# monniert/differentiable-blocksworld

Measured on AMD Instinct MI355X. Metric: rendered views/sec (fwd+bwd) per node, DTU 400x300 K=10 blocks, higher is better.
Workload: dtype f32; 1 GPU; DTU-scan24-like synthetic: 49 views/GPU/step, 400x300, 10 superquadric blocks + ground + sky dome, faces_per_pixel=10, 256^2 textures, coarse phase (sigma=1e-4, opacity noise, decimated textures), MSE+parsimony+TV+overlap, Adam; LPIPS excluded; views_per_gpu=49, n_blocks=10, faces_per_pixel=10, txt_size=256, parallelism=one GPU: all views on it, no collective, nranks=1

## Files before the change

### differentiable-blocksworld_amd/csrc/project_clip.hip

```cpp
#include "dbw_common.h"
#include "camera_math.h"
#include "shade_common.h"
#include "raster_bin.h"
#include "step_kernels.h"
#include "texture_body.h"
#include "../../include/dbw_hip.h"

using namespace dbw;

namespace {

constexpr int NT = 256;

__device__ __forceinline__ void store_tri(float *dst, f3 a, f3 b, f3 c) {
    dst[0] = a.x; dst[1] = a.y; dst[2] = a.z;
    dst[3] = b.x; dst[4] = b.y; dst[5] = b.z;
    dst[6] = c.x; dst[7] = c.y; dst[8] = c.z;
}

__global__ __launch_bounds__(NT) void project_clip_fwd_kernel(
    const float *__restrict__ verts, const int *__restrict__ faces, const float *__restrict__ R,
    const float *__restrict__ T, const float *__restrict__ Kmat, int V, int F, float eps, int zc_on, float zc,
    int persp, float *__restrict__ fvc, int *__restrict__ first_idx, int *__restrict__ num_faces,
    int *__restrict__ c2o, int *__restrict__ neighbor, int *__restrict__ code, float *__restrict__ cw) {
    __shared__ int s_wcnt[NT / DBW_WAVE];
    const int b = blockIdx.x, tid = threadIdx.x, lane = tid & 63, wv = tid >> 6;
    Cam cam;
    load_cam(R, T, Kmat, b, cam);
    const long long base_out = (long long)b * 2 * F;
    int running = 0;
    for (int f0 = 0; f0 < F; f0 += NT) {
        const int f = f0 + tid;
        ClippedFace cf;
        cf.emit = 0;
        if (f < F) {
            f3 p[3];
#pragma unroll
            for (int i = 0; i < 3; ++i) p[i] = project(verts + (long long)faces[f * 3 + i] * 3, cam, eps).ndc;
            clip_face(p, zc_on, zc, persp, cf);
        }
        const int emit = cf.emit;
        const unsigned long long m1 = __ballot(emit >= 1), m2 = __ballot(emit == 2);
        const unsigned long long lower = (1ull << lane) - 1ull;
        const int prefix = __popcll(m1 & lower) + __popcll(m2 & lower);
        if (lane == 0) s_wcnt[wv] = __popcll(m1) + __popcll(m2);
        __syncthreads();
        int woff = 0, tot = 0;
#pragma unroll
        for (int w = 0; w < NT / DBW_WAVE; ++w) { const int c = s_wcnt[w]; if (w < wv) woff += c; tot += c; }
        const int slot = running + woff + prefix;
        if (emit >= 1) {
            const long long o = base_out + slot;
            store_tri(fvc + o * 9, cf.t0[0], cf.t0[1], cf.t0[2]);
            c2o[o] = f; neighbor[o] = emit == 2 ? (int)(o + 1) : -1; code[o] = cf.code0; cw[o * 2] = cf.w2; cw[o * 2 + 1] = cf.w3;
            if (emit == 2) {
                store_tri(fvc + (o + 1) * 9, cf.t1[0], cf.t1[1], cf.t1[2]);
                c2o[o + 1] = f; neighbor[o + 1] = (int)o; code[o + 1] = cf.code1; cw[(o + 1) * 2] = cf.w2; cw[(o + 1) * 2 + 1] = cf.w3;
            }
        }
        running += tot;
        __syncthreads();
    }
    if (tid == 0) { first_idx[b] = (int)base_out; num_faces[b] = running; }
}

constexpr int BWD_SLOTS = 8;
template <bool LDS_TABLE>
__device__ __forceinline__ void project_clip_bwd_body(
    const float *__restrict__ verts, const int *__restrict__ faces, const float *__restrict__ R,
    const float *__restrict__ T, const float *__restrict__ Kmat, int B, int V, int F, float eps, float zc, int persp,
    const int *__restrict__ num_faces, const int *__restrict__ c2o, const int *__restrict__ code,
    const float *__restrict__ cw, const float *__restrict__ gfvc, float *gverts, float *s_acc, int blk) {
    const int lane = threadIdx.x & 63;
    if (LDS_TABLE) {
        for (int i = threadIdx.x; i < V * 3; i += NT) s_acc[i] = 0.f;
        __syncthreads();
    }
    constexpr int WAVES = NT / DBW_WAVE, ITERS = LDS_TABLE ? BWD_SLOTS / WAVES : 1;
    for (int it = 0; it < ITERS; ++it) {
    const int j = LDS_TABLE ? blk * BWD_SLOTS + it * WAVES + (threadIdx.x >> 6) : blk * WAVES + (threadIdx.x >> 6);
    if (j >= 2 * F) break;
    for (int b0 = 0; b0 < B; b0 += DBW_WAVE) {
        const int b = b0 + lane;
        bool act = b < B && j < num_faces[b];
        const long long o = (long long)(act ? b : 0) * 2 * F + j;
        float g[9];
        if (act) {
            bool any = false;
#pragma unroll
            for (int i = 0; i < 9; ++i) { g[i] = gfvc[o * 9 + i]; any |= (g[i] != 0.f); }
            act = any;
        }
        int f = -1, vi[3] = {0, 0, 0};
        float gw[9] = {0.f, 0.f, 0.f, 0.f, 0.f, 0.f, 0.f, 0.f, 0.f};
        if (act) {
            Cam cam;
            load_cam(R, T, Kmat, b, cam);
            f = c2o[o];
            const int cd = code[o];
            vi[0] = faces[f * 3]; vi[1] = faces[f * 3 + 1]; vi[2] = faces[f * 3 + 2];
            f3 gv[3] = {{0.f, 0.f, 0.f}, {0.f, 0.f, 0.f}, {0.f, 0.f, 0.f}};
            const f3 ga{g[0], g[1], g[2]}, gb{g[3], g[4], g[5]}, gc{g[6], g[7], g[8]};
            if (cd < 0) {
                gv[0] = ga; gv[1] = gb; gv[2] = gc;
            } else {
                const int i1 = cd & 3, kind = cd >> 2;
                const f3 q0 = project(verts + (long long)vi[0] * 3, cam, eps).ndc, q1 = project(verts + (long long)vi[1] * 3, cam, eps).ndc,
                         q2 = project(verts + (long long)vi[2] * 3, cam, eps).ndc;
                const f3 P1 = i1 == 0 ? q0 : (i1 == 1 ? q1 : q2), P2 = i1 == 0 ? q1 : (i1 == 1 ? q2 : q0),
                         P3 = i1 == 0 ? q2 : (i1 == 1 ? q0 : q1);
                const float w2 = cw[o * 2], w3 = cw[o * 2 + 1];
                f3 g1{0.f, 0.f, 0.f}, g2{0.f, 0.f, 0.f}, g3{0.f, 0.f, 0.f};
                if (kind == 0) {
                    clip_point_bwd(P1, P2, zc, persp, w2, ga, g1, g2);
                    clip_point_bwd(P1, P3, zc, persp, w3, gb, g1, g3);
                    g1.x += gc.x; g1.y += gc.y; g1.z += gc.z;
                } else if (kind == 1) {
                    clip_point_bwd(P1, P2, zc, persp, w2, ga, g1, g2);
                    g2.x += gb.x; g2.y += gb.y; g2.z += gb.z;
                    clip_point_bwd(P1, P3, zc, persp, w3, gc, g1, g3);
                } else {
                    clip_point_bwd(P1, P3, zc, persp, w3, ga, g1, g3);
                    g2.x += gb.x; g2.y += gb.y; g2.z += gb.z;
                    g3.x += gc.x; g3.y += gc.y; g3.z += gc.z;
                }
                gv[0] = i1 == 0 ? g1 : (i1 == 1 ? g3 : g2);
                gv[1] = i1 == 0 ? g2 : (i1 == 1 ? g1 : g3);
                gv[2] = i1 == 0 ? g3 : (i1 == 1 ? g2 : g1);
            }
#pragma unroll
            for (int i = 0; i < 3; ++i)
                if (gv[i].x != 0.f || gv[i].y != 0.f || gv[i].z != 0.f) {
                    const f3 w = vertex_bwd(verts, vi[i], cam, eps, gv[i]);
                    gw[i * 3] = w.x; gw[i * 3 + 1] = w.y; gw[i * 3 + 2] = w.z;
                }
        }
        const unsigned long long am = __ballot(act);
        if (am == 0ull) continue;
        const int leader = __ffsll((long long)am) - 1;
        const int f0 = __shfl(f, leader, 64);
        if (__popcll(am) >= 4 && __ballot(act && f == f0) == am) {
            float s[9];
#pragma unroll
            for (int c = 0; c < 9; ++c) s[c] = wave_sum_dpp(gw[c]);
            if (lane == leader) {
#pragma unroll
                for (int c = 0; c < 9; ++c)
                    if (s[c] != 0.f) {
                        if (LDS_TABLE) atomicAdd(&s_acc[vi[c / 3] * 3 + (c % 3)], s[c]);
                        else unsafeAtomicAdd(gverts + (long long)vi[c / 3] * 3 + (c % 3), s[c]);
                    }
            }
        } else if (act) {
#pragma unroll
            for (int c = 0; c < 9; ++c)
                if (gw[c] != 0.f) {
                    if (LDS_TABLE) atomicAdd(&s_acc[vi[c / 3] * 3 + (c % 3)], gw[c]);
                    else unsafeAtomicAdd(gverts + (long long)vi[c / 3] * 3 + (c % 3), gw[c]);
                }
        }
    }
    }
    if (LDS_TABLE) {
        __syncthreads();
        for (int i = threadIdx.x; i < V * 3; i += NT) {
            const float v = s_acc[i];
            if (v != 0.f) unsafeAtomicAdd(gverts + i, v);
        }
    }
}

template <bool LDS_TABLE>
__global__ __launch_bounds__(NT) void project_clip_bwd_kernel(
    const float *__restrict__ verts, const int *__restrict__ faces, const float *__restrict__ R,
    const float *__restrict__ T, const float *__restrict__ Kmat, int B, int V, int F, float eps, float zc, int persp,
    const int *__restrict__ num_faces, const int *__restrict__ c2o, const int *__restrict__ code,
    const float *__restrict__ cw, const float *__restrict__ gfvc, float *__restrict__ gverts) {
    extern __shared__ float s_acc[];
    project_clip_bwd_body<LDS_TABLE>(verts, faces, R, T, Kmat, B, V, F, eps, zc, persp, num_faces, c2o, code, cw, gfvc, gverts, s_acc, blockIdx.x);
}

template <bool LDS_TABLE>
__global__ __launch_bounds__(NT) void clip_bwd_tex_kernel(const ClipBwdArgs C, const dbw_texture_set t, int nclip) {
    extern __shared__ float s_acc[];
    if ((int)blockIdx.x < nclip)
        project_clip_bwd_body<LDS_TABLE>(C.verts, C.faces, C.R, C.T, C.Kmat, C.B, C.V, C.F, C.eps, C.zc, C.persp, C.num_faces, C.c2o, C.code, C.cw, C.gfvc,
                                         C.gverts, s_acc, blockIdx.x);
    else
        texture_prep_bwd_body(t.texture, t.n, t.h, t.w, t.decim, t.grad_maps, t.grad_sig, t.grad_texture, (long long)blockIdx.x - nclip,
                              (long long)gridDim.x - nclip);
}

template <bool CACHED>
__global__ __launch_bounds__(NT) void scene_setup_kernel(const SceneSetupArgs A) {
    __shared__ int s_wcnt[NT / DBW_WAVE];
    extern __shared__ float s_ndc[];
    if (A.sync_flag && blockIdx.x == 0 && blockIdx.y == 0 && blockIdx.z == 0 && threadIdx.x == 0)
        __hip_atomic_store(A.sync_flag, A.sync_val, __ATOMIC_RELEASE, __HIP_MEMORY_SCOPE_AGENT);
    const SceneGeom &G = A.sc[A.scene0 + blockIdx.z];
    const int chunk = blockIdx.x, b = blockIdx.y, tid = threadIdx.x, lane = tid & 63, wv = tid >> 6;
    const int F = G.F, nchunks = (F + NT - 1) / NT;
    if (chunk >= nchunks) return;
    if (G.hdr && chunk == 0 && b == 0)
        for (int i = tid; i < G.nhdr; i += NT) G.hdr[i] = 0;
    Cam cam;
    load_cam(A.R, A.T, A.Kmat, b, cam);
    const long long base_out = (long long)b * 2 * F;
    const int f = chunk * NT + tid;
    int vi[3] = {0, 0, 0};
    if (f < F) { vi[0] = G.faces[f * 3]; vi[1] = G.faces[f * 3 + 1]; vi[2] = G.faces[f * 3 + 2]; }
    if (CACHED) {
        for (int v = tid; v < G.V; v += NT) {
            const f3 q = project(G.verts + (long long)v * 3, cam, G.cam_eps).ndc;
            s_ndc[v * 3] = q.x; s_ndc[v * 3 + 1] = q.y; s_ndc[v * 3 + 2] = q.z;
        }
        __syncthreads();
    }
    int before = 0;
    for (int g = tid; g < chunk * NT; g += NT) {
        const int i0 = G.faces[g * 3], i1 = G.faces[g * 3 + 1], i2 = G.faces[g * 3 + 2];
        float z0, z1, z2;
        if (CACHED) { z0 = s_ndc[i0 * 3 + 2]; z1 = s_ndc[i1 * 3 + 2]; z2 = s_ndc[i2 * 3 + 2]; }
        else { z0 = view_z(G.verts + (long long)i0 * 3, cam); z1 = view_z(G.verts + (long long)i1 * 3, cam); z2 = view_z(G.verts + (long long)i2 * 3, cam); }
        before += clip_emit_count(z0, z1, z2, G.zc_on, G.zc);
    }
#pragma unroll
    for (int o = 32; o > 0; o >>= 1) before += __shfl_xor(before, o, 64);
    if (lane == 0) s_wcnt[wv] = before;
    __syncthreads();
    int running = 0;
#pragma unroll
    for (int w = 0; w < NT / DBW_WAVE; ++w) running += s_wcnt[w];
    __syncthreads();
    ClippedFace cf;
    cf.emit = 0;
    if (f < F) {
        f3 p[3];
#pragma unroll
        for (int i = 0; i < 3; ++i) {
            if (CACHED) p[i] = f3{s_ndc[vi[i] * 3], s_ndc[vi[i] * 3 + 1], s_ndc[vi[i] * 3 + 2]};
            else p[i] = project(G.verts + (long long)vi[i] * 3, cam, G.cam_eps).ndc;
        }
        clip_face(p, G.zc_on, G.zc, G.persp, cf);
    }
    const int emit = cf.emit;
    const unsigned long long m1 = __ballot(emit >= 1), m2 = __ballot(emit == 2);
    const unsigned long long lower = (1ull << lane) - 1ull;
    const int prefix = __popcll(m1 & lower) + __popcll(m2 & lower);
    if (lane == 0) s_wcnt[wv] = __popcll(m1) + __popcll(m2);
    __syncthreads();
    int woff = 0, tot = 0;
#pragma unroll
    for (int w = 0; w < NT / DBW_WAVE; ++w) { const int c = s_wcnt[w]; if (w < wv) woff += c; tot += c; }
    const int slot = running + woff + prefix;
    FaceRec *recs = (FaceRec *)G.recs;
    ShadeRec *srec = (ShadeRec *)G.srec;
#pragma unroll
    for (int t = 0; t < 2; ++t) {
        if (t >= emit) break;
        const long long o = base_out + slot + t;
        const f3 a = t == 0 ? cf.t0[0] : cf.t1[0], bq = t == 0 ? cf.t0[1] : cf.t1[1], cq = t == 0 ? cf.t0[2] : cf.t1[2];
        const float p9[9] = {a.x, a.y, a.z, bq.x, bq.y, bq.z, cq.x, cq.y, cq.z};
        const int nbr = emit == 2 ? (int)(t == 0 ? o + 1 : o - 1) : -1, cd = t == 0 ? cf.code0 : cf.code1;
#pragma unroll
        for (int i = 0; i < 9; ++i) G.fvc[o * 9 + i] = p9[i];
        G.c2o[o] = f; G.neighbor[o] = nbr; G.code[o] = cd; G.cw[o * 2] = cf.w2; G.cw[o * 2 + 1] = cf.w3;
        FaceRec r;
        float box[4];
        make_face_rec(p9, G.margin, 0, nbr, r, box);
        G.bbox[o] = make_float4(box[0], box[1], box[2], box[3]);
        recs[o] = r;
        if (srec) {
            ShadeRec sr;
            const float *uv = G.face_uvs + (long long)f * 6;
#pragma unroll
            for (int i = 0; i < 6; ++i) sr.uv[i] = uv[i];
            sr.j = f; sr.cd = cd; sr.w2 = cf.w2; sr.w3 = cf.w3;
            sr.map = G.face_map[f];
            sr.fa = G.map_alpha ? G.map_alpha[sr.map] : 1.f;
            const int *md = G.map_desc + sr.map * 8;
            sr.off = md[0]; sr.hw = (md[1] << 16) | md[2]; sr.pads = (md[3] << 16) | md[4]; sr.sh = md[5];
            srec[o] = sr;
        }
    }
    if (chunk == nchunks - 1 && tid == 0) {
        G.first_idx[b] = (int)base_out;
        G.num_faces[b] = running + tot;
        if (srec && b == 0 && running + tot == 0) {
            ShadeRec sr;
#pragma unroll
            for (int i = 0; i < 6; ++i) sr.uv[i] = 0.f;
            sr.j = 0; sr.cd = -1; sr.w2 = sr.w3 = 0.f; sr.map = 0; sr.fa = 0.f; sr.off = 0; sr.hw = (1 << 16) | 1; sr.pads = 0; sr.sh = 0;
            srec[0] = sr;
        }
    }
}

}

int dbw::launch_clip_bwd_tex(const ClipBwdArgs &C, const dbw_texture_set &t, hipStream_t s) {
    DBW_REQUIRE(C.verts && C.faces && C.R && C.T && C.Kmat && C.num_faces && C.c2o && C.code && C.cw && C.gfvc && C.gverts, "null pointer");
    DBW_REQUIRE(C.B > 0 && C.V > 0 && C.F > 0, "bad size");
    DBW_REQUIRE(t.texture && t.grad_maps && t.grad_texture && t.n > 0 && t.h > 0 && t.w > 0 && t.decim >= 1, "bad texture set");
    const long long work = (long long)t.n * t.h * t.w * 3;
    long long ntex = (work + NT - 1) / NT;
    if (ntex > 4096) ntex = 4096;
    const bool table = (size_t)C.V * 3 * sizeof(float) <= 48 * 1024;
    const int nclip = table ? (2 * C.F + BWD_SLOTS - 1) / BWD_SLOTS : (2 * C.F + NT / DBW_WAVE - 1) / (NT / DBW_WAVE);
    if (table)
        hipLaunchKernelGGL(clip_bwd_tex_kernel<true>, dim3((unsigned)(nclip + ntex)), dim3(NT), (size_t)C.V * 3 * sizeof(float), s, C, t, nclip);
    else
        hipLaunchKernelGGL(clip_bwd_tex_kernel<false>, dim3((unsigned)(nclip + ntex)), dim3(NT), 0, s, C, t, nclip);
    return dbw_check_launch("clip_bwd_tex_kernel");
}

int dbw::launch_scene_setup(const SceneSetupArgs &A, hipStream_t s) {
    DBW_REQUIRE(A.R && A.T && A.Kmat && A.B > 0, "bad argument");
    int chunks = 0;
    DBW_REQUIRE(A.scene0 >= 0 && A.nscenes >= 1 && A.scene0 + A.nscenes <= 2, "bad scene range");
    for (int i = A.scene0; i < A.scene0 + A.nscenes; ++i) {
        const SceneGeom &G = A.sc[i];
        DBW_REQUIRE(G.verts && G.faces && G.fvc && G.first_idx && G.num_faces && G.c2o && G.neighbor && G.code && G.cw && G.bbox && G.recs, "null pointer");
        DBW_REQUIRE(G.V > 0 && G.F > 0 && (long long)A.B * 2 * G.F < 0x7fffffffLL && (!G.zc_on || G.zc > 0.f), "bad size / z_clip");
        DBW_REQUIRE(!G.srec || (G.face_uvs && G.face_map && G.map_desc), "null pointer");
        chunks = max(chunks, (G.F + NT - 1) / NT);
    }
    int vmax = 0;
    for (int i = A.scene0; i < A.scene0 + A.nscenes; ++i) vmax = max(vmax, A.sc[i].V);
    if ((size_t)vmax * 12 <= 40 * 1024)
        hipLaunchKernelGGL(scene_setup_kernel<true>, dim3((unsigned)chunks, (unsigned)A.B, (unsigned)A.nscenes), dim3(NT), (size_t)vmax * 12, s, A);
    else
        hipLaunchKernelGGL(scene_setup_kernel<false>, dim3((unsigned)chunks, (unsigned)A.B, (unsigned)A.nscenes), dim3(NT), 0, s, A);
    return dbw_check_launch("scene_setup_kernel");
}

extern "C" int dbw_project_clip_fwd(const float *verts_world, const int32_t *faces, const float *R, const float *T,
                                    const float *Kmat, int B, int V, int F, float eps, int z_clip_enabled,
                                    float z_clip, int perspective_correct, float *face_verts_c, int32_t *first_idx,
                                    int32_t *num_faces, int32_t *c2o, int32_t *neighbor, int32_t *clip_code,
                                    float *clip_w, dbw_stream_t stream) {
    DBW_REQUIRE(verts_world && faces && R && T && Kmat && face_verts_c && first_idx && num_faces && c2o && neighbor &&
                    clip_code && clip_w, "null pointer");
    DBW_REQUIRE(B >= 0 && V > 0 && F > 0, "bad size");
    DBW_REQUIRE((long long)B * 2 * F < 0x7fffffffLL, "B*2F overflows int32 face indices");
    DBW_REQUIRE(!z_clip_enabled || z_clip > 0.f, "z_clip must be > 0");
    if (B == 0) return DBW_OK;
    hipLaunchKernelGGL(project_clip_fwd_kernel, dim3(B), dim3(NT), 0, (hipStream_t)stream, verts_world, faces, R, T,
                       Kmat, V, F, eps, z_clip_enabled, z_clip, perspective_correct, face_verts_c, first_idx,
                       num_faces, c2o, neighbor, clip_code, clip_w);
    return dbw_check_launch("project_clip_fwd_kernel");
}

extern "C" int dbw_project_clip_bwd(const float *verts_world, const int32_t *faces, const float *R, const float *T,
                                    const float *Kmat, int B, int V, int F, float eps, float z_clip,
                                    int perspective_correct, const int32_t *num_faces, const int32_t *c2o,
                                    const int32_t *clip_code, const float *clip_w, const float *grad_face_verts_c,
                                    float *grad_verts_world, dbw_stream_t stream) {
    DBW_REQUIRE(verts_world && faces && R && T && Kmat && num_faces && c2o && clip_code && clip_w &&
                    grad_face_verts_c && grad_verts_world, "null pointer");
    DBW_REQUIRE(B >= 0 && V > 0 && F > 0, "bad size");
    if (B == 0) return DBW_OK;
    if ((size_t)V * 3 * sizeof(float) <= 48 * 1024)
        hipLaunchKernelGGL(project_clip_bwd_kernel<true>, dim3((2 * F + BWD_SLOTS - 1) / BWD_SLOTS), dim3(NT), (size_t)V * 3 * sizeof(float),
                           (hipStream_t)stream, verts_world, faces, R, T, Kmat, B, V, F, eps, z_clip, perspective_correct, num_faces, c2o,
                           clip_code, clip_w, grad_face_verts_c, grad_verts_world);
    else
        hipLaunchKernelGGL(project_clip_bwd_kernel<false>, dim3((2 * F + NT / DBW_WAVE - 1) / (NT / DBW_WAVE)), dim3(NT), 0, (hipStream_t)stream,
                           verts_world, faces, R, T, Kmat, B, V, F, eps, z_clip, perspective_correct, num_faces, c2o,
                           clip_code, clip_w, grad_face_verts_c, grad_verts_world);
    return dbw_check_launch("project_clip_bwd_kernel");
}
```

### differentiable-blocksworld_amd/csrc/step_kernels.h

```cpp
#pragma once
#include <hip/hip_runtime.h>
#include <stdint.h>

#include "../../include/dbw_hip.h"

namespace dbw {
struct RasterWorkspace;

constexpr int STEP_MAX_SETS = 4;
struct StepTextureSets { dbw_texture_set s[STEP_MAX_SETS]; };

struct PrologueArgs {
    StepTextureSets tex; int nsets;
    const float *alpha_logit, *noise;
    float noise_scale, thresh;
    int nb;
    float *alpha, *alpha_full;
    int *keep;
    unsigned long long seed, rng_step;
    const float *sq_eps, *S, *R6, *T, *trig;
    int nv;
    float ratio, scale_min, S_world;
    const float *Rw, *Tw;
    float *blk_verts;
    float *sq_local;
    const float *ground_base; int ngv;
    const float *R6g, *Tg;
    float *ground_verts;
    float *zero0; int nzero0;
};
int launch_step_prologue(const PrologueArgs &P, hipStream_t s);

struct SceneGeom {
    const float *verts; const int *faces; int V, F;
    float cam_eps; int zc_on; float zc; int persp;
    float *fvc; int *first_idx, *num_faces, *c2o, *neighbor, *code; float *cw;
    float margin;
    float4 *bbox; void *recs;
    int *hdr; int nhdr;
    void *srec; const float *face_uvs; const int *face_map, *map_desc; const float *map_alpha;
};
struct SceneSetupArgs { SceneGeom sc[2]; const float *R, *T, *Kmat; int B; int scene0, nscenes;
                        unsigned *sync_flag; unsigned sync_val; };
int launch_scene_setup(const SceneSetupArgs &A, hipStream_t s);

struct SceneBinsArgs {
    struct One {
        const float4 *bbox; const void *recs; const int *first_idx, *num_faces;
        int *list, *count; unsigned *mask;
        int cells; int2 *cell; int *pool; int pool_cap; int *hdr; int *rank;
        int *dom;
    } sc[2];
    int B, H, W, nx, ny;
    int scene0, nscenes;
    StepTextureSets tex; int tex_sets, tex_z;
};
int launch_scene_bins(const SceneBinsArgs &A, hipStream_t s);
int dbw_launch_work_scatter(const RasterWorkspace &L, int N, int H, int W, hipStream_t s, unsigned *sync_flag = nullptr, unsigned sync_val = 0);

struct RegulariserArgs {
    const float *u; int npts;
    unsigned long long seed, rng_step;
    const float *sq_eps, *S, *R6, *T, *alpha_full;
    int nb;
    float ratio, scale_min, inv_temp, thresh, overlap_scale;
    float pars_eps, pars_scale;
    float *loss_parsimony, *loss_overlap;
    float *g_sq_eps, *g_S, *g_R6, *g_T, *g_alpha_full;
    float *ws;
    unsigned *ticket;
};
int launch_regularisers(const RegulariserArgs &A, hipStream_t s);

struct BlocksTailArgs {
    const float *sq_eps, *S, *R6, *T, *sq_local; const int *keep; int nb, nv; float scale_min, S_world; const float *Rw;
    const float *g_verts;
    float *g_sq_eps, *g_S, *g_R6, *g_T;
    const float *alpha, *g_alpha_parts, *g_alpha_full; int alpha_parts; float *g_logit;
    const float *void_raised; float *void_flag;
};
int launch_blocks_tail(const BlocksTailArgs &A, hipStream_t s);

struct ClipBwdArgs {
    const float *verts; const int *faces; const float *R, *T, *Kmat; int B, V, F; float eps, zc; int persp;
    const int *num_faces, *c2o, *code; const float *cw, *gfvc; float *gverts;
};
int launch_clip_bwd_tex(const ClipBwdArgs &C, const dbw_texture_set &tex, hipStream_t s);

struct AdamTailArgs {
    float *param, *grad, *exp_avg, *exp_avg_sq; const int64_t *group_end; const float *lr; int ngroups;
    float beta1, beta2, eps; int step;
    void *zero_buf; int64_t zero_bytes, hole_begin, hole_end;
    dbw_texture_set tex[2]; int ntex;
    const float *void_raised; float *void_flag;
};
bool adam_tail_fits(const AdamTailArgs &A);
int launch_adam_tail(const AdamTailArgs &A, hipStream_t s);

struct EnvFoldHost {
    const RasterWorkspace *ws; const int *first_idx, *num_faces; const float *maps; float bg[3];
    int *p2f; float *uvj;
};
int render_fwd_fused_mse_fold(const float *face_verts_c, const int32_t *first_idx, const int32_t *num_faces, const int32_t *neighbor,
                              const int32_t *c2o, const int32_t *clip_code, const float *clip_w, int Fc_stride, const float *face_uvs,
                              const int32_t *face_map, const int32_t *map_desc, const float *maps, const float *faces_alpha, int alpha_len, int N,
                              int64_t F_total, int H, int W, int K, int F, float sigma, float blur_radius, int perspective_correct,
                              const float *background3, int32_t *pix_to_face, float *bary, float *dists, void *workspace, size_t workspace_bytes,
                              const float *target, float mse_scale, float *loss_partial, float *grad_fg, float *grad_env, const EnvFoldHost &fold,
                              float *rec_out, const float *grad_rec, hipStream_t stream);

int render_bwd_fused_signal(const int32_t *pix_to_face, const float *bary, const float *dists, const int32_t *c2o, const int32_t *clip_code,
                            const float *clip_w, int Fc_stride, const float *face_uvs, const int32_t *face_map, const int32_t *map_desc, const float *maps,
                            const float *faces_alpha, int alpha_len, int N, int H, int W, int K, int F, float sigma, const float *background3,
                            const float *grad_image, const float *face_verts_c, int perspective_correct, int detach_bary, float *grad_maps,
                            float *grad_faces_alpha, float *grad_face_verts_c, int lds_aggregate, int frag_layout, const int32_t *bin_base,
                            int32_t *bin_cursor, void *bin_records, int bin_cap, const uint32_t *bin_layout, int const_geometry_faces,
                            const float *grad_scale, int image_layout, dbw_stream_t stream, unsigned *sync_flag, unsigned sync_val);

}
```

### differentiable-blocksworld_amd/csrc/texture.hip

```cpp
#include "dbw_common.h"
#include "loss_math.h"
#include "texture_body.h"
#include "step_kernels.h"
#include "../../include/dbw_hip.h"

#include <string.h>
#include <algorithm>

using namespace dbw;

namespace {

constexpr int NT = 256;

__device__ __forceinline__ float sigmoidf(float x) { return 1.f / (1.f + expf(-x)); }

__device__ __forceinline__ float block_sum(float v, float *s_red) {
    v = wave_sum(v);
    const int lane = threadIdx.x & 63, wv = threadIdx.x >> 6;
    __syncthreads();
    if (lane == 0) s_red[wv] = v;
    __syncthreads();
    float t = 0.f;
#pragma unroll
    for (int w = 0; w < NT / DBW_WAVE; ++w) t += s_red[w];
    return t;
}

__global__ __launch_bounds__(256) void texture_prep_fwd_kernel(const float *__restrict__ tex, int n, int h, int w, int d,
                                                               float *__restrict__ maps, float *__restrict__ sig) {
    texture_prep_fwd_body(tex, n, h, w, d, maps, sig, blockIdx.x, gridDim.x);
}

constexpr int MAX_SETS = 4;
struct TextureSets { dbw_texture_set s[MAX_SETS]; };

__global__ __launch_bounds__(256) void texture_prep_fwd_sets_kernel(const TextureSets S) {
    const dbw_texture_set &t = S.s[blockIdx.y];
    texture_prep_fwd_body(t.texture, t.n, t.h, t.w, t.decim, t.maps, t.sig, blockIdx.x, gridDim.x);
}

__global__ void texture_prep_bwd_kernel(const float *__restrict__ tex, int n, int h, int w, int d,
                                        const float *__restrict__ gmaps, const float *__restrict__ gsig,
                                        float *__restrict__ gtex) {
    texture_prep_bwd_body(tex, n, h, w, d, gmaps, gsig, gtex, blockIdx.x, gridDim.x);
}

__global__ void texture_prep_bwd_sets_kernel(const TextureSets S) {
    const dbw_texture_set &t = S.s[blockIdx.y];
    texture_prep_bwd_body(t.texture, t.n, t.h, t.w, t.decim, t.grad_maps, t.grad_sig, t.grad_texture, blockIdx.x, gridDim.x);
}

__device__ __forceinline__ void tv_l2sq_body(const float *__restrict__ m, int n, int h, int w, int wrap,
                                             float scale, float *__restrict__ loss, float *__restrict__ gm, float *s_red) {
    const float sx = 1.f / ((float)h * (float)(w - 1 + (wrap ? 1 : 0)));
    const float sy = 1.f / ((float)(h - 1) * (float)w);
    float part = 0.f;
    for (int row = blockIdx.y; row < n * h; row += gridDim.y) {
        const int y = row % h;
        const float *r = m + (long long)row * w * 3;
        for (int x = blockIdx.x * NT + threadIdx.x; x < w; x += gridDim.x * NT) {
            float g3[3];
            part += tv_l2sq_texel(r, x, y, w, h, wrap, sx, sy, g3);
            if (gm) {
#pragma unroll
                for (int c = 0; c < 3; ++c) gm[((long long)row * w + x) * 3 + c] = scale * g3[c];
            }
        }
    }
    const float tot = block_sum(part, s_red);
    if (threadIdx.x == 0 && tot != 0.f) unsafeAtomicAdd(loss, scale * tot);
}

__global__ __launch_bounds__(NT) void tv_l2sq_kernel(const float *__restrict__ m, int n, int h, int w, int wrap,
                                                     float scale, float *__restrict__ loss, float *__restrict__ gm) {
    __shared__ float s_red[NT / DBW_WAVE];
    tv_l2sq_body(m, n, h, w, wrap, scale, loss, gm, s_red);
}

__global__ __launch_bounds__(NT) void tv_l2sq_sets_kernel(const TextureSets S, float *__restrict__ loss) {
    __shared__ float s_red[NT / DBW_WAVE];
    const dbw_texture_set &t = S.s[blockIdx.z];
    tv_l2sq_body(t.sig, t.n, t.h, t.w, t.wrap_x, t.tv_scale, loss, t.grad_sig_out, s_red);
}

constexpr int CNT = 1024;
__global__ __launch_bounds__(CNT) void composite_mse_kernel(const float *__restrict__ fg, const float *__restrict__ env,
                                                           const float *__restrict__ img, int N, long long plane,
                                                           float scale, const float *__restrict__ scale_dev, float *__restrict__ rec,
                                                           float *__restrict__ loss, float *__restrict__ gfg,
                                                           float *__restrict__ genv) {
    __shared__ float s_red[CNT / DBW_WAVE];
    const long long total = (long long)N * plane;
    float part = 0.f;
    const float loss_scale = scale;
    if (scale_dev) scale *= scale_dev[0];
    for (long long i0 = (long long)blockIdx.x * CNT; i0 < total; i0 += (long long)gridDim.x * CNT) {
        const long long i = i0 + threadIdx.x;
        if (i < total) {
            const long long n = i / plane, p = i % plane;
            const float *f = fg + n * 4 * plane + p, *e = env + n * 4 * plane + p;
            const float *t = img ? img + n * 3 * plane + p : nullptr;
            const float mask = f[3 * plane];
            const float fc3[3] = {f[0], f[plane], f[2 * plane]}, ec3[3] = {e[0], e[plane], e[2 * plane]};
            const float t3[3] = {t ? t[0] : 0.f, t ? t[plane] : 0.f, t ? t[2 * plane] : 0.f};
            float rec3[3], gf3[3], ge3[3], gmask = 0.f;
            part += composite_mse_pixel(fc3, mask, ec3, t3, t != nullptr, 2.f * scale, rec3, gf3, ge3, gmask);
#pragma unroll
            for (int c = 0; c < 3; ++c) {
                if (rec) rec[n * 3 * plane + c * plane + p] = rec3[c];
                if (gfg) { gfg[n * 4 * plane + c * plane + p] = gf3[c]; genv[n * 4 * plane + c * plane + p] = ge3[c]; }
            }
            if (gfg) { gfg[n * 4 * plane + 3 * plane + p] = gmask; genv[n * 4 * plane + 3 * plane + p] = 0.f; }
        }
    }
    part = wave_sum(part);
    if ((threadIdx.x & 63) == 0) s_red[threadIdx.x >> 6] = part;
    __syncthreads();
    if (threadIdx.x == 0 && loss) {
        float tot = 0.f;
        for (int w = 0; w < CNT / DBW_WAVE; ++w) tot += s_red[w];
        unsafeAtomicAdd(loss, tot * loss_scale);
    }
}

__global__ void adam_kernel(float *__restrict__ p, const float *__restrict__ g, float *__restrict__ m,
                            float *__restrict__ v, long long n, float step_size, float beta1, float beta2, float eps,
                            float bc2_sqrt) {
    for (long long i = (long long)blockIdx.x * blockDim.x + threadIdx.x; i < n; i += (long long)gridDim.x * blockDim.x) {
        adam_update(p[i], g[i], m[i], v[i], step_size, beta1, beta2, eps, bc2_sqrt);
    }
}

struct AdamGroups { long long end[MAX_SETS]; float step_size[MAX_SETS]; };

__global__ void adam_groups_kernel(float *__restrict__ p, const float *__restrict__ g, float *__restrict__ m, float *__restrict__ v,
                                   long long n, const AdamGroups G, float beta1, float beta2, float eps, float bc2_sqrt,
                                   uint4 *__restrict__ zero_buf, long long zero_vec, const float *__restrict__ skip_flag) {
    if (skip_flag && *skip_flag != 0.f) n = 0;
    for (long long i = (long long)blockIdx.x * blockDim.x + threadIdx.x; i < n; i += (long long)gridDim.x * blockDim.x) {
        float step_size = G.step_size[0];
#pragma unroll
        for (int k = 1; k < MAX_SETS; ++k) step_size = i >= G.end[k - 1] ? G.step_size[k] : step_size;
        adam_update(p[i], g[i], m[i], v[i], step_size, beta1, beta2, eps, bc2_sqrt);
    }
    for (long long i = (long long)blockIdx.x * blockDim.x + threadIdx.x; i < zero_vec; i += (long long)gridDim.x * blockDim.x)
        zero_buf[i] = make_uint4(0u, 0u, 0u, 0u);
}

__device__ __forceinline__ float group_step_size(const AdamGroups &G, long long i) {
    float step_size = G.step_size[0];
#pragma unroll
    for (int k = 1; k < MAX_SETS; ++k) step_size = i >= G.end[k - 1] ? G.step_size[k] : step_size;
    return step_size;
}

struct AdamTex { const float *tex; const float *gsig; float *gmaps; int n, h, w, d; long long off; };
struct AdamTailK {
    float *p, *g, *m, *v; long long n; AdamGroups G; float beta1, beta2, eps, bc2_sqrt;
    uint4 *zero_buf; long long zero_vec, hole_lo, hole_hi;
    AdamTex t[2]; int ntex, clear_maps, nenv;
    long long skip_lo[2], skip_len[2];
    const float *void_raised; float *void_flag;
};

__device__ __forceinline__ void adam_tex_set(const AdamTailK &A, const AdamTex &t, bool skip, long long etid, long long neth) {
    if (t.d <= 1) {
        const long long total = (long long)t.n * t.h * t.w * 3;
        for (long long i = etid; i < total; i += neth) {
            const float s = tex_sigmoid(t.tex[i]);
            float g = t.gmaps[i];
            if (A.clear_maps) t.gmaps[i] = 0.f;
            if (t.gsig) g += t.gsig[i];
            const float gt = g * s * (1.f - s);
            const long long o = t.off + i;
            A.g[o] = gt;
            if (!skip) adam_update(A.p[o], gt, A.m[o], A.v[o], group_step_size(A.G, o), A.beta1, A.beta2, A.eps, A.bc2_sqrt);
        }
        return;
    }
    const float inv = 1.f / (float)(t.d * t.d);
    const int ch_ = t.h / t.d, cw_ = t.w / t.d, lane = threadIdx.x & 63;
    const long long cells = (long long)t.n * ch_ * cw_;
    for (long long c = etid >> 6; c < cells; c += neth >> 6) {
        const int m = (int)(c / ((long long)ch_ * cw_));
        const int r = (int)(c % ((long long)ch_ * cw_));
        const int cy = r / cw_, cx = r % cw_;
        const float gc[3] = {t.gmaps[c * 3], t.gmaps[c * 3 + 1], t.gmaps[c * 3 + 2]};
        for (int q = lane; q < t.d * t.d; q += 64) {
            const long long e = (((long long)m * t.h + cy * t.d + q / t.d) * t.w + cx * t.d + q % t.d) * 3;
#pragma unroll
            for (int ch = 0; ch < 3; ++ch) {
                const long long i = e + ch;
                const float s = tex_sigmoid(t.tex[i]);
                float g = gc[ch] * inv;
                if (t.gsig) g += t.gsig[i];
                const float gt = g * s * (1.f - s);
                const long long o = t.off + i;
                A.g[o] = gt;
                if (!skip) adam_update(A.p[o], gt, A.m[o], A.v[o], group_step_size(A.G, o), A.beta1, A.beta2, A.eps, A.bc2_sqrt);
            }
        }
        if (A.clear_maps && lane < 3) t.gmaps[c * 3 + lane] = 0.f;
    }
}

__global__ __launch_bounds__(NT) void adam_groups_tex_kernel(const AdamTailK A) {
    const bool skip = *A.void_raised != 0.f;
    if (blockIdx.x == 0 && threadIdx.x == 0 && A.void_flag) *A.void_flag = *A.void_raised;
    const long long tid = (long long)blockIdx.x * blockDim.x + threadIdx.x, nth = (long long)gridDim.x * blockDim.x;
    const long long neth = (long long)A.nenv * blockDim.x;
    if (tid < neth) {
        for (int k = 0; k < A.ntex; ++k) adam_tex_set(A, A.t[k], skip, tid, neth);
    } else if (!skip) {
        const long long rest = A.n - A.skip_len[0] - A.skip_len[1];
        for (long long j = tid - neth; j < rest; j += nth - neth) {
            long long i = j;
            if (i >= A.skip_lo[0]) i += A.skip_len[0];
            if (i >= A.skip_lo[1]) i += A.skip_len[1];
            adam_update(A.p[i], A.g[i], A.m[i], A.v[i], group_step_size(A.G, i), A.beta1, A.beta2, A.eps, A.bc2_sqrt);
        }
    }
    for (long long i = tid; i < A.zero_vec; i += nth)
        if (i < A.hole_lo || i >= A.hole_hi) A.zero_buf[i] = make_uint4(0u, 0u, 0u, 0u);
}

inline unsigned grid_for(long long work) {
    long long b = (work + NT - 1) / NT;
    if (b < 1) b = 1;
    if (b > 2048) b = 2048;
    return (unsigned)b;
}

}

extern "C" int dbw_texture_prep_fwd(const float *texture, int n, int h, int w, int decim, float *maps_out,
                                    float *sig_out, dbw_stream_t stream) {
    DBW_REQUIRE(texture && maps_out, "null pointer");
    DBW_REQUIRE(n > 0 && h > 0 && w > 0 && decim >= 1, "bad size");
    DBW_REQUIRE(decim == 1 || sig_out, "sig_out is required when decimating");
    DBW_REQUIRE(decim == 1 || (h % decim == 0 && w % decim == 0), "map size must be a multiple of the decimation factor");
    const long long work = decim > 1 ? (long long)n * (h / decim) * (w / decim) * 64 : (long long)n * h * w * 3;
    hipLaunchKernelGGL(texture_prep_fwd_kernel, dim3(grid_for(work)), dim3(NT), 0, (hipStream_t)stream, texture, n, h,
                       w, decim, maps_out, sig_out);
    return dbw_check_launch("texture_prep_fwd_kernel");
}

extern "C" int dbw_texture_prep_bwd(const float *texture, int n, int h, int w, int decim, const float *grad_maps,
                                    const float *grad_sig, float *grad_texture, dbw_stream_t stream) {
    DBW_REQUIRE(texture && grad_maps && grad_texture, "null pointer");
    DBW_REQUIRE(n > 0 && h > 0 && w > 0 && decim >= 1, "bad size");
    DBW_REQUIRE(decim == 1 || (h % decim == 0 && w % decim == 0), "map size must be a multiple of the decimation factor");
    const long long work = (long long)n * h * w * 3;
    hipLaunchKernelGGL(texture_prep_bwd_kernel, dim3(grid_for(work)), dim3(NT), 0, (hipStream_t)stream, texture, n, h,
                       w, decim, grad_maps, grad_sig, grad_texture);
    return dbw_check_launch("texture_prep_bwd_kernel");
}

extern "C" int dbw_tv_l2sq(const float *maps, int n, int h, int w, int wrap_x, float scale, float *loss,
                           float *grad_maps, dbw_stream_t stream) {
    DBW_REQUIRE(maps && loss, "null pointer");
    DBW_REQUIRE(n > 0 && h > 1 && w > 1, "bad size");
    const long long rows = (long long)n * h;
    hipLaunchKernelGGL(tv_l2sq_kernel, dim3((unsigned)((w + NT - 1) / NT), (unsigned)(rows < 512 ? rows : 512)), dim3(NT), 0,
                       (hipStream_t)stream, maps, n, h, w, wrap_x, scale, loss, grad_maps);
    return dbw_check_launch("tv_l2sq_kernel");
}

namespace {
int check_sets(const dbw_texture_set *sets, int nsets) {
    DBW_REQUIRE(sets && nsets >= 1 && nsets <= MAX_SETS, "1..4 texture sets");
    for (int i = 0; i < nsets; ++i) {
        const dbw_texture_set &t = sets[i];
        DBW_REQUIRE(t.n > 0 && t.h > 1 && t.w > 1 && t.decim >= 1, "bad size");
        DBW_REQUIRE(t.decim == 1 || (t.h % t.decim == 0 && t.w % t.decim == 0), "map size must be a multiple of the decimation factor");
    }
    return DBW_OK;
}
TextureSets pack_sets(const dbw_texture_set *sets, int nsets) {
    TextureSets S;
    for (int i = 0; i < MAX_SETS; ++i) S.s[i] = sets[i < nsets ? i : 0];
    return S;
}
AdamGroups adam_groups(const int64_t *group_end, const float *lr, int ngroups, float beta1, float beta2, int step, float &bc2_sqrt) {
    const long long n = group_end[ngroups - 1];
    const double bc1 = 1.0 - pow((double)beta1, step), bc2 = 1.0 - pow((double)beta2, step);
    AdamGroups G;
    for (int k = 0; k < MAX_SETS; ++k) {
        G.end[k] = k < ngroups ? group_end[k] : n;
        G.step_size[k] = (float)(lr[k < ngroups ? k : ngroups - 1] / bc1);
    }
    bc2_sqrt = (float)sqrt(bc2);
    return G;
}
}

extern "C" int dbw_texture_prep_fwd_sets(const dbw_texture_set *sets, int nsets, dbw_stream_t stream) {
    if (int rc = check_sets(sets, nsets)) return rc;
    long long work = 0;
    for (int i = 0; i < nsets; ++i) {
        const dbw_texture_set &t = sets[i];
        DBW_REQUIRE(t.texture && t.maps, "null pointer");
        DBW_REQUIRE(t.decim == 1 || t.sig, "sig is required when decimating");
        const long long wk = t.decim > 1 ? (long long)t.n * (t.h / t.decim) * (t.w / t.decim) * 64 : (long long)t.n * t.h * t.w * 3;
        work = wk > work ? wk : work;
    }
    hipLaunchKernelGGL(texture_prep_fwd_sets_kernel, dim3(grid_for(work), (unsigned)nsets), dim3(NT), 0, (hipStream_t)stream,
                       pack_sets(sets, nsets));
    return dbw_check_launch("texture_prep_fwd_sets_kernel");
}

extern "C" int dbw_texture_prep_bwd_sets(const dbw_texture_set *sets, int nsets, dbw_stream_t stream) {
    if (int rc = check_sets(sets, nsets)) return rc;
    long long work = 0;
    for (int i = 0; i < nsets; ++i) {
        const dbw_texture_set &t = sets[i];
        DBW_REQUIRE(t.texture && t.grad_maps && t.grad_texture, "null pointer");
        const long long wk = (long long)t.n * t.h * t.w * 3;
        work = wk > work ? wk : work;
    }
    hipLaunchKernelGGL(texture_prep_bwd_sets_kernel, dim3(grid_for(work), (unsigned)nsets), dim3(NT), 0, (hipStream_t)stream,
                       pack_sets(sets, nsets));
    return dbw_check_launch("texture_prep_bwd_sets_kernel");
}

extern "C" int dbw_tv_l2sq_sets(const dbw_texture_set *sets, int nsets, float *loss, dbw_stream_t stream) {
    if (int rc = check_sets(sets, nsets)) return rc;
    DBW_REQUIRE(loss, "null pointer");
    long long rows = 0;
    int w = 0;
    for (int i = 0; i < nsets; ++i) {
        DBW_REQUIRE(sets[i].sig, "null pointer");
        const long long r = (long long)sets[i].n * sets[i].h;
        rows = r > rows ? r : rows;
        w = sets[i].w > w ? sets[i].w : w;
    }
    hipLaunchKernelGGL(tv_l2sq_sets_kernel, dim3((unsigned)((w + NT - 1) / NT), (unsigned)(rows < 512 ? rows : 512), (unsigned)nsets),
                       dim3(NT), 0, (hipStream_t)stream, pack_sets(sets, nsets), loss);
    return dbw_check_launch("tv_l2sq_sets_kernel");
}

extern "C" int dbw_adam_step_groups(float *param, const float *grad, float *exp_avg, float *exp_avg_sq, const int64_t *group_end,
                                    const float *lr, int ngroups, float beta1, float beta2, float eps, int step, void *zero_buf,
                                    int64_t zero_bytes, const float *skip_flag, dbw_stream_t stream) {
    DBW_REQUIRE(param && grad && exp_avg && exp_avg_sq && group_end && lr, "null pointer");
    DBW_REQUIRE(zero_bytes >= 0 && (zero_bytes == 0 || (zero_buf && zero_bytes % 16 == 0 && ((uintptr_t)zero_buf & 15) == 0)),
                "zero_buf: 16-byte aligned, a multiple of 16 bytes");
    DBW_REQUIRE(ngroups >= 1 && ngroups <= MAX_SETS && step >= 1, "1..4 groups, step >= 1");
    for (int k = 0; k < ngroups; ++k) DBW_REQUIRE(group_end[k] >= (k ? group_end[k - 1] : 0), "group ends must not decrease");
    const long long n = group_end[ngroups - 1];
    if (n == 0) return DBW_OK;
    float bc2_sqrt;
    const AdamGroups G = adam_groups(group_end, lr, ngroups, beta1, beta2, step, bc2_sqrt);
    hipLaunchKernelGGL(adam_groups_kernel, dim3(grid_for(n)), dim3(NT), 0, (hipStream_t)stream, param, grad, exp_avg, exp_avg_sq, n, G,
                       beta1, beta2, eps, bc2_sqrt, (uint4 *)zero_buf, (long long)(zero_bytes / 16), skip_flag);
    return dbw_check_launch("adam_groups_kernel");
}

bool dbw::adam_tail_fits(const AdamTailArgs &A) {
    if (!A.param || !A.grad || !A.exp_avg || !A.exp_avg_sq || !A.group_end || !A.lr || !A.void_raised || A.ngroups < 1 || A.ngroups > MAX_SETS) return false;
    if (A.ntex < 0 || A.ntex > 2 || A.zero_bytes < 0 || A.zero_bytes % 16 || ((uintptr_t)A.zero_buf & 15)) return false;
    if (A.hole_begin < 0 || A.hole_begin > A.hole_end || A.hole_end > A.zero_bytes || A.hole_begin % 16 || A.hole_end % 16) return false;
    const long long n = A.group_end[A.ngroups - 1];
    const char *hb = (const char *)A.zero_buf + A.hole_begin, *he = (const char *)A.zero_buf + A.hole_end;
    long long lo[2] = {0, 0}, hi[2] = {0, 0};
    for (int k = 0; k < A.ntex; ++k) {
        const dbw_texture_set &t = A.tex[k];
        if (!t.texture || !t.grad_maps || !t.grad_texture || t.n < 1 || t.h < 1 || t.w < 1 || t.decim < 1 || t.h % t.decim || t.w % t.decim) return false;
        lo[k] = (long long)(t.grad_texture - A.grad);
        hi[k] = lo[k] + (long long)t.n * t.h * t.w * 3;
        if (t.grad_texture < A.grad || hi[k] > n || t.texture != A.param + lo[k]) return false;
        const char *mb = (const char *)t.grad_maps, *me = mb + (size_t)t.n * (t.h / t.decim) * (t.w / t.decim) * 3 * sizeof(float);
        const char *zb = (const char *)A.zero_buf, *ze = zb + A.zero_bytes;
        if (A.hole_end > A.hole_begin ? (mb < hb || me > he) : (mb < ze && me > zb)) return false;
    }
    return A.ntex < 2 || hi[0] <= lo[1] || hi[1] <= lo[0];
}

int dbw::launch_adam_tail(const AdamTailArgs &A, hipStream_t s) {
    DBW_REQUIRE(adam_tail_fits(A), "the texture sets must lie in the flat buffers, their maps' gradients in the hole of the arena");
    DBW_REQUIRE(A.step >= 1, "step >= 1");
    for (int k = 0; k < A.ngroups; ++k) DBW_REQUIRE(A.group_end[k] >= (k ? A.group_end[k - 1] : 0), "group ends must not decrease");
    AdamTailK K;
    memset(&K, 0, sizeof(K));
    K.p = A.param; K.g = A.grad; K.m = A.exp_avg; K.v = A.exp_avg_sq; K.n = A.group_end[A.ngroups - 1];
    K.G = adam_groups(A.group_end, A.lr, A.ngroups, A.beta1, A.beta2, A.step, K.bc2_sqrt);
    K.beta1 = A.beta1; K.beta2 = A.beta2; K.eps = A.eps;
    K.zero_buf = (uint4 *)A.zero_buf; K.zero_vec = A.zero_bytes / 16; K.hole_lo = A.hole_begin / 16; K.hole_hi = A.hole_end / 16;
    K.ntex = A.ntex; K.clear_maps = A.hole_end > A.hole_begin ? 1 : 0;
    for (int k = 0; k < A.ntex; ++k) {
        const dbw_texture_set &t = A.tex[k];
        K.t[k].tex = t.texture; K.t[k].gsig = t.grad_sig; K.t[k].gmaps = (float *)t.grad_maps;
        K.t[k].n = t.n; K.t[k].h = t.h; K.t[k].w = t.w; K.t[k].d = t.decim; K.t[k].off = (long long)(t.grad_texture - A.grad);
    }
    K.void_raised = A.void_raised; K.void_flag = A.void_flag;
    long long env = 0;
    for (int k = 0; k < 2; ++k) {
        K.skip_lo[k] = K.n; K.skip_len[k] = 0;
        if (k < A.ntex) { K.skip_lo[k] = K.t[k].off; K.skip_len[k] = (long long)K.t[k].n * K.t[k].h * K.t[k].w * 3; env += K.skip_len[k]; }
    }
    if (K.skip_lo[1] < K.skip_lo[0]) {
        std::swap(K.skip_lo[0], K.skip_lo[1]);
        std::swap(K.skip_len[0], K.skip_len[1]);
    }
    unsigned grid = grid_for(K.n);
    K.nenv = 0;
    if (A.ntex) {
        if (grid < 2) grid = 2;
        const double we = 10.0 / 7.0 * (double)env;
        const long long share = (long long)((double)grid * we / ((double)(K.n - env) + we) + 0.5);
        K.nenv = (int)std::min<long long>(grid - 1, std::max<long long>(1, share));
    }
    hipLaunchKernelGGL(adam_groups_tex_kernel, dim3(grid), dim3(NT), 0, s, K);
    return dbw_check_launch("adam_groups_tex_kernel");
}

extern "C" int dbw_debug_adam_tail(float *param, float *grad, float *exp_avg, float *exp_avg_sq, const int64_t *group_end, const float *lr,
                                   int ngroups, float beta1, float beta2, float eps, int step, void *zero_buf, int64_t zero_bytes,
                                   int64_t hole_begin, int64_t hole_end, const dbw_texture_set *sets, int nsets, const float *void_raised,
                                   float *void_flag, dbw_stream_t stream) {
    DBW_REQUIRE(nsets >= 0 && nsets <= 2 && (sets || nsets == 0), "0..2 texture sets");
    AdamTailArgs A;
    memset(&A, 0, sizeof(A));
    A.param = param; A.grad = grad; A.exp_avg = exp_avg; A.exp_avg_sq = exp_avg_sq; A.group_end = group_end; A.lr = lr; A.ngroups = ngroups;
    A.beta1 = beta1; A.beta2 = beta2; A.eps = eps; A.step = step;
    A.zero_buf = zero_buf; A.zero_bytes = zero_bytes; A.hole_begin = hole_begin; A.hole_end = hole_end;
    for (int k = 0; k < nsets; ++k) A.tex[k] = sets[k];
    A.ntex = nsets; A.void_raised = void_raised; A.void_flag = void_flag;
    return launch_adam_tail(A, (hipStream_t)stream);
}

extern "C" int dbw_composite_mse(const float *fg, const float *env, const float *imgs, int N, int H, int W,
                                 float scale, const float *scale_dev, float *rec, float *loss_sum, float *grad_fg,
                                 float *grad_env, dbw_stream_t stream) {
    DBW_REQUIRE(fg && env, "null pointer");
    DBW_REQUIRE(imgs || (!loss_sum && !grad_fg && rec), "imgs may only be NULL when just `rec` is wanted");
    DBW_REQUIRE((grad_fg && grad_env) || (!grad_fg && !grad_env), "grad_fg/grad_env: both or none");
    DBW_REQUIRE(N >= 0 && H > 0 && W > 0, "bad size");
    if (N == 0) return DBW_OK;
    const long long plane = (long long)H * W;
    long long gb = ((long long)N * plane + CNT - 1) / CNT;
    if (gb > 512) gb = 512;
    hipLaunchKernelGGL(composite_mse_kernel, dim3((unsigned)(gb < 1 ? 1 : gb)), dim3(CNT), 0, (hipStream_t)stream, fg,
                       env, imgs, N, plane, scale, scale_dev, rec, loss_sum, grad_fg, grad_env);
    return dbw_check_launch("composite_mse_kernel");
}

extern "C" int dbw_adam_step(float *param, const float *grad, float *exp_avg, float *exp_avg_sq, int64_t n, float lr,
                             float beta1, float beta2, float eps, int step, dbw_stream_t stream) {
    DBW_REQUIRE(param && grad && exp_avg && exp_avg_sq, "null pointer");
    DBW_REQUIRE(n >= 0 && step >= 1, "bad size/step");
    if (n == 0) return DBW_OK;
    const double bc1 = 1.0 - pow((double)beta1, step), bc2 = 1.0 - pow((double)beta2, step);
    hipLaunchKernelGGL(adam_kernel, dim3(grid_for(n)), dim3(NT), 0, (hipStream_t)stream, param, grad, exp_avg,
                       exp_avg_sq, (long long)n, (float)(lr / bc1), beta1, beta2, eps, (float)sqrt(bc2));
    return dbw_check_launch("adam_kernel");
}
```

### differentiable-blocksworld_amd/csrc/train_step.hip

```cpp
#include "dbw_common.h"
#include "raster_bin.h"
#include "step_kernels.h"
#include "../../include/dbw_hip.h"

#include <math.h>
#include <mutex>
#include <new>
#include <stdlib.h>
#include <string.h>

using namespace dbw;

namespace {

__global__ __launch_bounds__(256) void tile_target_kernel(const float *__restrict__ img, int B, int C, int H, int W, float *__restrict__ out) {
    const int tx = (W + 7) >> 3, ty = (H + 7) >> 3;
    const long long total = (long long)B * ty * tx * C * 64;
    for (long long i = (long long)blockIdx.x * blockDim.x + threadIdx.x; i < total; i += (long long)gridDim.x * blockDim.x) {
        const int lane = (int)(i & 63);
        long long r = i >> 6;
        const int c = (int)(r % C); r /= C;
        const int tix = (int)(r % tx); r /= tx;
        const int tiy = (int)(r % ty);
        const int n = (int)(r / ty);
        const int y = tiy * 8 + (lane >> 3), x = tix * 8 + (lane & 7);
        out[i] = (y < H && x < W) ? img[(((long long)n * C + c) * H + y) * W + x] : 0.f;
    }
}

constexpr int LOSS_BLOCKS = 32;
__global__ __launch_bounds__(256) void loss_finish_kernel(const float *__restrict__ part, long long nparts, float scale, float tv_value_scale, float *vals,
                                                          float *__restrict__ out5) {
    __shared__ float s_red[4];
    __shared__ int s_last;
    float acc = 0.f;
    for (long long i = (long long)blockIdx.x * 256 + threadIdx.x; i < nparts; i += (long long)gridDim.x * 256) acc += part[i];
    acc = wave_sum(acc);
    if ((threadIdx.x & 63) == 0) s_red[threadIdx.x >> 6] = acc;
    __syncthreads();
    if (threadIdx.x == 0) {
        const float t = (s_red[0] + s_red[1]) + (s_red[2] + s_red[3]);
        if (t != 0.f) unsafeAtomicAdd(vals, t);
        __threadfence();
        s_last = atomicAdd((unsigned *)(vals + 5), 1u) == gridDim.x - 1 ? 1 : 0;
    }
    __syncthreads();
    if (s_last && threadIdx.x == 0) {
        __threadfence();
        const float rgb = atomicAdd(vals, 0.f) * scale;
        const float tvv = vals[2] * tv_value_scale;
        out5[0] = rgb; out5[1] = vals[1]; out5[2] = tvv; out5[3] = vals[3];
        out5[4] = ((rgb + vals[1]) + tvv) + vals[3];
    }
}

size_t al(size_t x) { return (x + 255) & ~(size_t)255; }

struct SceneBuf { size_t fvc, first, num, c2o, nbr, code, cw, rws, rws_bytes; };

struct Layout {
    SceneBuf e, f;
    size_t p2f_e, bary_e, dists_e, img_e, p2f, bary, dists, part, g_fg, g_env;
    size_t env_maps, blk_maps, sig[3], g_sig[3];
    size_t alpha, alpha_full, keep, blk_verts, sq_local, losses, target;
    size_t records, cursor[2], layout[2], layout_uniform;
    size_t arena_begin, g_alpha_full, ovl_ws, vals, tickets, g_blk_maps, g_env_maps, g_maps_end, g_fa, g_fvc_f, g_blk_verts, g_fvc_e, g_env_verts, arena_end;
    size_t total;
    int Fe, Ff, Ve, Vf, tiles, bin_cap;
    size_t ce, cb_, n_env_maps, n_blk_maps;
};

bool tv_on(const dbw_step_desc &d) { return d.w_tv_bkg != 0.f || d.w_tv_blocks != 0.f || d.w_tv_ground != 0.f; }
bool bins_on(const dbw_step_desc &d) { return d.decim_blocks == 1 && d.n_bins > 0 && d.block_bin_base && d.block_bin_info; }

int texbin_capacity(int B, int H, int W, int K, int nbins) {
    long long cap = (long long)B * H * W * (K > 4 ? K : 4) / (2LL * nbins);
    if (cap < 256) cap = 256;
    const long long hi = (16LL << 30) / (32LL * nbins);
    if (cap > hi) cap = hi;
    return (int)((cap + DBW_BIN_SUBCURSORS - 1) / DBW_BIN_SUBCURSORS * DBW_BIN_SUBCURSORS);
}

void scene_layout(SceneBuf &s, size_t &o, int B, int F, int H, int W) {
    const size_t n = (size_t)B * 2 * F;
    s.fvc = o; o += al(n * 9 * 4);
    s.first = o; o += al((size_t)B * 4);
    s.num = o; o += al((size_t)B * 4);
    s.c2o = o; o += al(n * 4);
    s.nbr = o; o += al(n * 4);
    s.code = o; o += al(n * 4);
    s.cw = o; o += al(n * 8);
    s.rws_bytes = dbw_rasterize_workspace_bytes_binned((int64_t)n, B, H, W);
    s.rws = o; o += al(s.rws_bytes);
}

void make_layout(const dbw_step_desc &d, Layout &L) {
    memset(&L, 0, sizeof(L));
    const int B = d.max_views, K = d.faces_per_pixel;
    L.Fe = d.n_sky_faces + d.n_ground_faces; L.Ff = d.n_blocks * d.block_nf;
    L.Ve = d.n_sky_verts + d.n_ground_verts; L.Vf = d.n_blocks * d.block_nv;
    L.tiles = ((d.H + 7) / 8) * ((d.W + 7) / 8);
    const size_t bt = (size_t)B * L.tiles;
    L.ce = (size_t)(d.env_txt_size / d.decim_env) * (d.env_txt_size / d.decim_env) * 3;
    L.cb_ = (size_t)(d.txt_size / d.decim_blocks) * (d.txt_size / d.decim_blocks) * 3;
    L.n_env_maps = 2 * L.ce; L.n_blk_maps = (size_t)d.n_blocks * L.cb_;
    size_t o = 0;
    scene_layout(L.e, o, B, L.Fe, d.H, d.W);
    scene_layout(L.f, o, B, L.Ff, d.H, d.W);
    L.p2f_e = o; o += al(bt * 64 * 4);
    L.bary_e = o; o += al(bt * 64 * 3 * 4);
    L.dists_e = o; o += al(bt * 64 * 4);
    L.img_e = o; o += al(bt * 256 * 4);
    L.p2f = o; o += al(bt * K * 64 * 4);
    L.bary = o; o += al(bt * K * 64 * 8 * 4);
    L.dists = o; o += al(bt * K * 64 * 4);
    L.part = o; o += al(bt * 4);
    L.g_fg = o; o += al(bt * 256 * 4);
    L.g_env = o; o += al(bt * 256 * 4);
    L.env_maps = o; o += al(L.n_env_maps * 4);
    L.blk_maps = o; o += al(L.n_blk_maps * 4);
    const size_t full[3] = {(size_t)d.env_txt_size * d.env_txt_size * 3, (size_t)d.n_blocks * d.txt_size * d.txt_size * 3, (size_t)d.env_txt_size * d.env_txt_size * 3};
    const int dec[3] = {d.decim_env, d.decim_blocks, d.decim_env};
    for (int i = 0; i < 3; ++i) {
        if (dec[i] > 1) { L.sig[i] = o; o += al(full[i] * 4); }
        else L.sig[i] = i == 0 ? L.env_maps : (i == 1 ? L.blk_maps : L.env_maps + L.ce * 4);
        if (tv_on(d)) { L.g_sig[i] = o; o += al(full[i] * 4); }
    }
    L.alpha = o; o += al((size_t)d.n_blocks * 4);
    L.alpha_full = o; o += al((size_t)d.n_blocks * 4);
    L.keep = o; o += al((size_t)d.n_blocks * 4);
    L.blk_verts = o; o += al((size_t)L.Vf * 12);
    L.sq_local = o; o += al((size_t)L.Vf * 36);
    L.losses = o; o += al(8 * 4);
    L.target = o; o += al(bt * 192 * 4);
    if (bins_on(d)) {
        L.bin_cap = texbin_capacity(B, d.H, d.W, K, d.n_bins);
        const size_t nsub = (size_t)d.n_bins * DBW_BIN_SUBCURSORS;
        L.records = o; o += al((size_t)d.n_bins * L.bin_cap * 32);
        for (int i = 0; i < 2; ++i) { L.cursor[i] = o; o += al(nsub * 4); }
        for (int i = 0; i < 2; ++i) { L.layout[i] = o; o += al(nsub * 8); }
        L.layout_uniform = o; o += al(nsub * 8);
    }
    L.arena_begin = o;
    L.g_alpha_full = o; o += al((size_t)d.n_blocks * 4);
    L.ovl_ws = o; o += al((size_t)d.n_blocks * 18 * 4);
    L.vals = o; o += al(8 * 4);
    L.tickets = o; o += al(4 * 4);
    L.g_blk_maps = o; o += al(L.n_blk_maps * 4);
    L.g_env_maps = o; o += al(L.n_env_maps * 4);
    L.g_maps_end = o;
    L.g_fa = o; o += al((size_t)d.n_blocks * 64 * 4);
    L.g_fvc_f = o; o += al((size_t)B * 2 * L.Ff * 9 * 4);
    L.g_blk_verts = o; o += al((size_t)L.Vf * 12);
    L.g_fvc_e = o; o += al((size_t)B * 2 * L.Fe * 9 * 4);
    L.g_env_verts = o; o += al((size_t)L.Ve * 12);
    L.arena_end = o;
    L.total = o;
}


void fill_texture_sets(const dbw_step_desc &d, const Layout &L, char *ws, dbw_texture_set (&sets)[3]) {
#define FPW(off) ((float *)(ws + (off)))
    memset(sets, 0, sizeof(sets));
    const float *tex[3] = {d.texture_bkg, d.textures, d.texture_ground};
    float *gtex[3] = {d.g_texture_bkg, d.g_textures, d.g_texture_ground};
    const int tn[3] = {1, d.n_blocks, 1}, th[3] = {d.env_txt_size, d.txt_size, d.env_txt_size}, td[3] = {d.decim_env, d.decim_blocks, d.decim_env};
    float *maps_out[3] = {FPW(L.env_maps), FPW(L.blk_maps), FPW(L.env_maps) + L.ce};
    float *gmaps[3] = {FPW(L.g_env_maps), FPW(L.g_blk_maps), FPW(L.g_env_maps) + L.ce};
    const float tvw[3] = {d.w_tv_bkg, d.w_tv_blocks, d.w_tv_ground};
    for (int i = 0; i < 3; ++i) {
        dbw_texture_set &t = sets[i];
        t.texture = tex[i]; t.n = tn[i]; t.h = th[i]; t.w = th[i]; t.decim = td[i];
        t.maps = maps_out[i];
        t.sig = td[i] > 1 ? FPW(L.sig[i]) : nullptr;
        t.wrap_x = i == 1 ? 1 : 0;
        t.tv_scale = tvw[i];
        t.grad_texture = gtex[i];
        t.grad_maps = gmaps[i];
    }
}
void add_tv_fields(const Layout &L, char *ws, dbw_texture_set (&sets)[3]) {
    for (int i = 0; i < 3; ++i) {
        sets[i].sig = FPW(L.sig[i]);
        sets[i].grad_sig_out = FPW(L.g_sig[i]);
        sets[i].grad_sig = FPW(L.g_sig[i]);
    }
#undef FPW
}

int check_desc(const dbw_step_desc *d) {
    DBW_REQUIRE(d, "null descriptor");
    DBW_REQUIRE(d->H > 0 && d->W > 0 && d->max_views > 0 && d->faces_per_pixel > 1 && d->faces_per_pixel <= DBW_MAX_FACES_PER_PIXEL, "bad image size / batch / faces_per_pixel (the soft pass has K > 1)");
    DBW_REQUIRE(d->n_blocks > 0 && d->n_blocks <= 64 && d->block_nv > 0 && d->block_nf > 0, "1..64 blocks");
    DBW_REQUIRE(d->n_blocks * d->block_nf < (1 << 20) && d->n_blocks + 2 < (1 << 11), "uv-fragments pack the face in 20 bits, the map in 11");
    DBW_REQUIRE(d->n_sky_verts > 0 && d->n_ground_verts > 0 && d->n_sky_faces > 0 && d->n_ground_faces > 0, "bad env mesh");
    DBW_REQUIRE(d->txt_size > 1 && d->env_txt_size > 1 && d->decim_env >= 1 && d->decim_blocks >= 1 && d->txt_size % d->decim_blocks == 0 &&
                    d->env_txt_size % d->decim_env == 0, "texture sizes must be multiples of their decimation factor");
    DBW_REQUIRE(d->sigma > 0.f && d->blur_radius >= 0.f && d->cam_eps > 0.f, "bad renderer constants");
    DBW_REQUIRE(d->R_world && d->T_world && d->Kmat && d->ground_base && d->env_verts && d->env_faces && d->env_face_uvs && d->env_face_map && d->env_map_desc &&
                    d->trig && d->block_faces && d->block_face_uvs && d->block_face_map && d->block_map_desc, "null table");
    DBW_REQUIRE(d->sq_eps && d->S && d->R6 && d->T && d->alpha_logit && d->R6_ground && d->T_ground && d->texture_bkg && d->texture_ground && d->textures, "null parameter");
    DBW_REQUIRE(d->g_sq_eps && d->g_S && d->g_R6 && d->g_T && d->g_alpha_logit && d->g_R6_ground && d->g_T_ground && d->g_texture_bkg && d->g_texture_ground &&
                    d->g_textures, "null gradient");
    DBW_REQUIRE(d->flat_param && d->flat_grad && d->exp_avg && d->exp_avg_sq && d->group_end[0] >= 0 && d->group_end[1] >= d->group_end[0], "bad Adam buffers");
    DBW_REQUIRE(d->small_grads && d->n_small_grads > 0, "small_grads: the accumulated gradients to clear");
    DBW_REQUIRE(d->w_rgb > 0.f && d->w_parsimony >= 0.f && d->w_overlap >= 0.f && d->w_tv_bkg >= 0.f && d->w_tv_blocks >= 0.f && d->w_tv_ground >= 0.f, "bad loss weights");
    DBW_REQUIRE(d->w_overlap == 0.f || (d->overlap_points > 0 && d->overlap_temperature > 0.f), "bad overlap constants");
    DBW_REQUIRE(((size_t)(d->n_sky_verts + d->n_ground_verts) * 12 <= 48 * 1024 && (size_t)d->n_blocks * d->block_nv * 12 <= 48 * 1024) || !(d->fuse & 8),
                "fused tails keep a scene's vertex gradients in 48 KB of LDS");
    DBW_REQUIRE((size_t)d->n_blocks * d->txt_size * d->txt_size * 3 < ((size_t)1 << 30) &&
                    (size_t)2 * d->env_txt_size * d->env_txt_size * 3 < ((size_t)1 << 30), "a scene's prepared maps must hold fewer than 2^30 floats");
    return DBW_OK;
}

constexpr int MAX_DEVICES = 64;
hipStream_t g_stream_r[MAX_DEVICES], g_stream_env[MAX_DEVICES];
std::mutex g_stream_lock;
int step_streams(hipStream_t &r, hipStream_t &e) {
    std::lock_guard<std::mutex> hold(g_stream_lock);
    int dev = 0;
    if (hipGetDevice(&dev) != hipSuccess || dev < 0 || dev >= MAX_DEVICES) { dbw_set_error("dbw_train_step_create: no current device"); return DBW_ERR_LAUNCH; }
    if (!g_stream_r[dev]) {
        int least = 0, greatest = 0;
        (void)hipDeviceGetStreamPriorityRange(&least, &greatest);
        if (hipStreamCreateWithPriority(&g_stream_r[dev], hipStreamNonBlocking, least) != hipSuccess ||
            hipStreamCreateWithPriority(&g_stream_env[dev], hipStreamNonBlocking, least) != hipSuccess) {
            dbw_set_error("dbw_train_step_create: hipStreamCreate failed");
            return DBW_ERR_LAUNCH;
        }
    }
    r = g_stream_r[dev]; e = g_stream_env[dev];
    return DBW_OK;
}

constexpr int SYNC_FLAGS = 12, SYNC_TIMEOUT_SLOT = 15, SYNC_WORDS = 32;
constexpr int SYNC_VOID_SLOT = 28;
enum { F_PROLOGUE, F_SCATTER, F_FG_FWD, F_REG, F_LAYOUT, F_KERNEL_DONE, F_BLOCKS_READY, F_ENV_DONE, F_TEX };
__global__ void sync_set_kernel(unsigned *flag, unsigned v) { __hip_atomic_store(flag, v, __ATOMIC_RELEASE, __HIP_MEMORY_SCOPE_AGENT); }
__global__ void void_latch_kernel(const float *void_raised, float *void_flag) { *void_flag = *void_raised; }
__global__ void sync_wait_kernel(const unsigned *flag, unsigned v, unsigned *timeouts, unsigned *host_timeouts, float *void_flag, unsigned long long limit) {
    const unsigned long long t0 = wall_clock64();
    const unsigned long long min_spins = limit >> 8;
    unsigned long long spins = 0;
    while ((int)(__hip_atomic_load(flag, __ATOMIC_ACQUIRE, __HIP_MEMORY_SCOPE_AGENT) - v) < 0) {
        __builtin_amdgcn_s_sleep(2);
        if (++spins > min_spins && wall_clock64() - t0 > limit) {
            atomicAdd(timeouts, 1u);
            if (atomicCAS(timeouts - 3, 0u, (unsigned)(flag - (timeouts - SYNC_TIMEOUT_SLOT)) + 1u) == 0u) {
                timeouts[-2] = v;
                timeouts[-1] = __hip_atomic_load(flag, __ATOMIC_ACQUIRE, __HIP_MEMORY_SCOPE_AGENT);
                for (int i = 0; i < SYNC_FLAGS; ++i) timeouts[1 + i] = __hip_atomic_load(timeouts - SYNC_TIMEOUT_SLOT + i, __ATOMIC_ACQUIRE, __HIP_MEMORY_SCOPE_AGENT);
            }
            __hip_atomic_store(void_flag, 1.f, __ATOMIC_RELEASE, __HIP_MEMORY_SCOPE_AGENT);
            __hip_atomic_store(host_timeouts, 1u, __ATOMIC_RELEASE, __HIP_MEMORY_SCOPE_SYSTEM);
            break;
        }
    }
}
constexpr unsigned long long SYNC_LIMIT_TICKS = 100000000ull;

}

struct dbw_step_plan {
    dbw_step_desc d;
    Layout L;
    char *ws;
    RasterWorkspace rw_e, rw_f;
    hipEvent_t ev_prologue, ev_scatter, ev_fg_fwd, ev_reg, ev_layout, ev_kernel_done, ev_blocks_ready, ev_env_done, ev_losses;
    hipStream_t stream_r, stream_env;
    unsigned long long runs;
    int bin_turn, bin_ready, uniform_ready;
    bool arena_clean;
    float *host_losses;
    bool losses_pending;
    bool phase1_done;
    bool cur_flags;
    bool profile, profiled;
    hipEvent_t ev_t[8];
    unsigned *sync_words;
    unsigned *host_timeouts, *host_timeouts_dev;
    unsigned sync_val[SYNC_FLAGS];
    int voided_runs;
    int force_timeout;
    bool last_tail;
};

extern "C" size_t dbw_train_step_workspace_bytes(const dbw_step_desc *desc) {
    if (check_desc(desc)) return 0;
    Layout L;
    make_layout(*desc, L);
    return L.total;
}

extern "C" dbw_step_plan *dbw_train_step_create(const dbw_step_desc *desc, void *workspace, size_t workspace_bytes) {
    if (check_desc(desc)) return nullptr;
    if (!workspace || ((uintptr_t)workspace & 255)) { dbw_set_error("dbw_train_step_create: the workspace must be 256-byte aligned"); return nullptr; }
    dbw_step_plan *p = new (std::nothrow) dbw_step_plan();
    if (!p) { dbw_set_error("dbw_train_step_create: out of host memory"); return nullptr; }
    p->d = *desc;
    make_layout(p->d, p->L);
    if (workspace_bytes < p->L.total) {
        dbw_set_error("dbw_train_step_create: workspace of %zu bytes, %zu needed", workspace_bytes, p->L.total);
        dbw_train_step_destroy(p);
        return nullptr;
    }
    p->ws = (char *)workspace;
    hipEvent_t *evs[] = {&p->ev_prologue, &p->ev_scatter, &p->ev_fg_fwd, &p->ev_reg, &p->ev_layout, &p->ev_kernel_done, &p->ev_blocks_ready, &p->ev_env_done, &p->ev_losses};
    for (hipEvent_t *e : evs)
        if (hipEventCreateWithFlags(e, hipEventDisableTiming) != hipSuccess) { dbw_set_error("dbw_train_step_create: hipEventCreate failed"); dbw_train_step_destroy(p); return nullptr; }
    if (step_streams(p->stream_r, p->stream_env)) { dbw_train_step_destroy(p); return nullptr; }
    if (hipHostMalloc((void **)&p->host_losses, 8 * sizeof(float), hipHostMallocDefault) != hipSuccess) {
        dbw_set_error("dbw_train_step_create: hipHostMalloc failed");
        dbw_train_step_destroy(p);
        return nullptr;
    }
    for (int i = 0; i < 8; ++i) p->host_losses[i] = 0.f;
    p->sync_words = nullptr;
    if (hipMalloc((void **)&p->sync_words, SYNC_WORDS * sizeof(unsigned)) != hipSuccess || hipMemset(p->sync_words, 0, SYNC_WORDS * sizeof(unsigned)) != hipSuccess) {
        dbw_set_error("dbw_train_step_create: hipMalloc failed");
        dbw_train_step_destroy(p);
        return nullptr;
    }
    for (unsigned &v : p->sync_val) v = 0;
    p->host_timeouts = nullptr; p->host_timeouts_dev = nullptr;
    if (hipHostMalloc((void **)&p->host_timeouts, 64, hipHostMallocMapped) != hipSuccess ||
        hipHostGetDevicePointer((void **)&p->host_timeouts_dev, p->host_timeouts, 0) != hipSuccess) {
        dbw_set_error("dbw_train_step_create: hipHostMalloc (mapped) failed");
        dbw_train_step_destroy(p);
        return nullptr;
    }
    *p->host_timeouts = 0u;
    p->profile = p->profiled = false;
    p->phase1_done = false;
    for (hipEvent_t &e : p->ev_t)
        if (hipEventCreate(&e) != hipSuccess) { dbw_set_error("dbw_train_step_create: hipEventCreate failed"); dbw_train_step_destroy(p); return nullptr; }
    p->runs = 0; p->cur_flags = false; p->voided_runs = 0; p->force_timeout = 0; p->bin_turn = 0; p->bin_ready = 0; p->uniform_ready = 0; p->arena_clean = false; p->losses_pending = false;
    p->last_tail = false;
    return p;
}

extern "C" void dbw_train_step_destroy(dbw_step_plan *p) {
    if (!p) return;
    hipEvent_t evs[] = {p->ev_prologue, p->ev_scatter, p->ev_fg_fwd, p->ev_reg, p->ev_layout, p->ev_kernel_done, p->ev_blocks_ready, p->ev_env_done, p->ev_losses};
    for (hipEvent_t e : evs) if (e) (void)hipEventDestroy(e);
    for (hipEvent_t e : p->ev_t) if (e) (void)hipEventDestroy(e);
    if (p->host_losses) (void)hipHostFree(p->host_losses);
    if (p->sync_words) (void)hipFree(p->sync_words);
    if (p->host_timeouts) (void)hipHostFree(p->host_timeouts);
    delete p;
}

extern "C" int64_t dbw_train_step_offset(const dbw_step_plan *p, int which) {
    if (!p) return -1;
    const Layout &L = p->L;
    switch (which) {
        case 0: return (int64_t)L.alpha;
        case 1: return (int64_t)L.alpha_full;
        case 2: return (int64_t)L.keep;
        case 3: return (int64_t)L.losses;
        case 4: return (int64_t)L.arena_begin;
        case 5: return (int64_t)L.arena_end;
        case 6: return (int64_t)L.g_fg;
        case 7: return (int64_t)L.g_env;
        case 8: return (int64_t)L.img_e;
        case 9: return (int64_t)L.blk_verts;
        case 10: return (int64_t)L.part;
        case 11: return (int64_t)L.p2f_e;
        case 12: return (int64_t)L.bary_e;
        case 13: return (int64_t)L.g_blk_maps;
        case 14: return (int64_t)L.g_maps_end;
        default: return -1;
    }
}


extern "C" int dbw_train_step_losses(dbw_step_plan *p, float *out5) {
    DBW_REQUIRE(p && out5, "null pointer");
    DBW_REQUIRE(p->losses_pending, "no run with read_losses != 0 to read from");
    if (hipEventSynchronize(p->ev_losses) != hipSuccess) { dbw_set_error("dbw_train_step_losses: hipEventSynchronize failed"); return DBW_ERR_LAUNCH; }
    for (int i = 0; i < 5; ++i) out5[i] = p->host_losses[i];
    return DBW_OK;
}

#define HIP_OK(call)                                                              \
    do {                                                                          \
        const hipError_t e_ = (call);                                             \
        if (e_ != hipSuccess) {                                                   \
            dbw_set_error("dbw_train_step_run: %s: %s", #call, hipGetErrorString(e_)); \
            return DBW_ERR_LAUNCH;                                                \
        }                                                                         \
    } while (0)
#define RC(call)                  \
    do {                          \
        const int rc_ = (call);   \
        if (rc_) return rc_;      \
    } while (0)

extern "C" int dbw_train_step_run(dbw_step_plan *p, const dbw_step_inputs *in, dbw_stream_t stream_main, dbw_stream_t stream_side) {
    DBW_REQUIRE(p && in, "null pointer");
    const dbw_step_desc &d = p->d;
    const Layout &L = p->L;
    DBW_REQUIRE(in->imgs && in->R && in->T, "null input");
    if (*(volatile unsigned *)p->host_timeouts != 0u) {
        HIP_OK(hipDeviceSynchronize());
        *(volatile unsigned *)p->host_timeouts = 0u;
        HIP_OK(hipMemset(p->sync_words + SYNC_VOID_SLOT, 0, sizeof(unsigned)));
        p->d.sync_events = 1;
        p->voided_runs += 1;
        p->arena_clean = false;
    }
    DBW_REQUIRE(in->B >= 1 && in->B <= d.max_views, "B must lie in [1, max_views]");
    DBW_REQUIRE(in->global_count > 0.0, "global_count must be positive");
    DBW_REQUIRE(!in->with_adam || in->adam_step >= 1, "adam_step >= 1");
    const bool defer = in->defer_textures != 0;
    DBW_REQUIRE(!defer || !in->with_adam, "defer_textures: Adam runs in dbw_train_step_finish");
    const int phase = in->phase;
    DBW_REQUIRE(phase >= 0 && phase <= 2 && (phase != 1 || in->rec_out) && (phase != 2 || in->grad_rec), "phase 1 stores rec_out, phase 2 reads grad_rec");
    DBW_REQUIRE(phase == 0 || ((p->d.fuse & 18) == 18), "the two-phase iteration (perceptual term) needs the env layer folded into the fg pass (fuse bits 1 and 4)");
    DBW_REQUIRE(phase != 2 || p->phase1_done, "phase 2 without a phase 1 in front of it");
    const bool head = phase != 2, rest = phase != 1;
    hipStream_t M = (hipStream_t)stream_main;
    const bool two = !in->single_stream;
    hipStream_t E = !two ? M : (stream_side ? (hipStream_t)stream_side : p->stream_env), Rg = two ? p->stream_r : M;
    if (head) p->cur_flags = d.sync_events == 0 && p->runs > 0;
    const bool flags = p->cur_flags;
    auto signal = [&](hipStream_t st, int idx, hipEvent_t ev) -> int {
        if (!flags) { HIP_OK(hipEventRecord(ev, st)); return DBW_OK; }
        hipLaunchKernelGGL(sync_set_kernel, dim3(1), dim3(1), 0, st, p->sync_words + idx, ++p->sync_val[idx]);
        return dbw_check_launch("sync_set_kernel");
    };
    char *ws = p->ws;
    float *void_flag = (float *)(ws + L.losses) + 7;
    float *void_raised = (float *)(p->sync_words + SYNC_VOID_SLOT);
    const int force_timeout = p->force_timeout;
    p->force_timeout = 0;
    auto await = [&](hipStream_t st, int idx, hipEvent_t ev) -> int {
        if (!flags) { HIP_OK(hipStreamWaitEvent(st, ev, 0)); return DBW_OK; }
        const bool forced = force_timeout == 1 && idx == F_ENV_DONE;
        const bool hasty = force_timeout == 2 && idx == F_PROLOGUE;
        hipLaunchKernelGGL(sync_wait_kernel, dim3(1), dim3(1), 0, st, (const unsigned *)(p->sync_words + idx), p->sync_val[idx] + (forced ? 0x10000000u : 0u),
                           p->sync_words + SYNC_TIMEOUT_SLOT, p->host_timeouts_dev, void_raised, forced ? 5000000ull : hasty ? 2000000ull : SYNC_LIMIT_TICKS);
        return dbw_check_launch("sync_wait_kernel");
    };
#define FP(off) ((float *)(ws + (off)))
#define IP(off) ((int *)(ws + (off)))
    const int B = in->B, H = d.H, W = d.W, K = d.faces_per_pixel, nb = d.n_blocks, nv = d.block_nv;
    const int Fe = L.Fe, Ff = L.Ff, Ve = L.Ve, Vf = L.Vf;
    const bool coarse = d.coarse != 0, bins = bins_on(d), tv = tv_on(d);
    const float mse_scale = (float)((double)d.w_rgb / in->global_count);
    const int zc_on = d.z_clip > 0.f ? 1 : 0;
    const bool noise_on = coarse && d.opacity_noise != 0.f;
    const float *fa = coarse ? FP(L.alpha) : nullptr;
    const int alpha_len = coarse ? -nb : 0;
    const int64_t Fte = (int64_t)B * 2 * Fe, Ftf = (int64_t)B * 2 * Ff;
    const bool overlap_on = d.w_overlap != 0.f, pars_on = d.w_parsimony != 0.f;
    DBW_REQUIRE((d.fuse & 1) || !noise_on || in->noise_override, "the operator-level prologue needs the caller's opacity noise (noise_override)");
    DBW_REQUIRE((d.fuse & 4) || !overlap_on || in->overlap_u_override, "the operator-level regularisers need the caller's overlap samples (overlap_u_override)");

    if (head && !p->arena_clean && !(in->arena_is_clean && p->runs > 0)) HIP_OK(hipMemsetAsync(ws + L.arena_begin, 0, L.arena_end - L.arena_begin, M));
    p->arena_clean = false;

    dbw_texture_set sets[3];
    fill_texture_sets(d, L, ws, sets);

    AdamTailArgs T;
    memset(&T, 0, sizeof(T));
    T.param = d.flat_param; T.grad = d.flat_grad; T.exp_avg = d.exp_avg; T.exp_avg_sq = d.exp_avg_sq; T.group_end = d.group_end; T.lr = in->lr;
    T.ngroups = 2; T.beta1 = in->beta1; T.beta2 = in->beta2; T.eps = in->adam_eps; T.step = in->adam_step;
    T.zero_buf = ws + L.arena_begin; T.zero_bytes = (int64_t)(L.arena_end - L.arena_begin);
    T.hole_begin = (int64_t)(L.g_env_maps - L.arena_begin); T.hole_end = (int64_t)(L.g_maps_end - L.arena_begin);
    T.tex[0] = sets[0]; T.tex[1] = sets[2]; T.ntex = 2;
    T.void_raised = void_raised; T.void_flag = void_flag;
    const bool adam_tail = in->with_adam && !defer && (d.fuse & 41) == 41 && two && in->B > d.serial_setup_max_views && !bins_on(d) &&
                           adam_tail_fits(T);

    const float *target = in->imgs;
    if (!in->imgs_tiled) {
        const long long total = (long long)B * L.tiles * 192;
        long long g = (total + 255) / 256;
        if (g > 4096) g = 4096;
        if (head) {
            hipLaunchKernelGGL(tile_target_kernel, dim3((unsigned)g), dim3(256), 0, M, in->imgs, B, 3, H, W, FP(L.target));
            RC(dbw_check_launch("tile_target_kernel"));
        }
        target = FP(L.target);
    }

    RasterWorkspace we, wf;
    RC(dbw_raster_workspace_layout(ws + L.e.rws, L.e.rws_bytes, Fte, 2 * Fe, B, H, W, (d.fuse & 16) != 0, we));
    RC(dbw_raster_workspace_layout(ws + L.f.rws, L.f.rws_bytes, Ftf, 2 * Ff, B, H, W, true, wf));
    const bool fused_setup = (d.fuse & 2) && we.binned && wf.binned && wf.cells;
    const bool fold = fused_setup && (d.fuse & 16) && we.cells;
    const float margin_f = (float)sqrt((double)d.blur_radius);
    const bool setup_aside = two && fused_setup && !fold && B > d.serial_setup_max_views;
    DBW_REQUIRE(phase == 0 || fold, "the two-phase iteration needs per-tile lists for both scenes (a binned workspace)");
    const bool tex_in_bins = (d.fuse & 64) && (d.fuse & 1) && flags && two && fused_setup && !setup_aside;
    const float thresh = d.mask_threshold;
    if (!head) {
    } else if (d.fuse & 1) {
        PrologueArgs P;
        memset(&P, 0, sizeof(P));
        for (int i = 0; i < 3; ++i) P.tex.s[i] = sets[i];
        P.tex.s[3] = sets[0];
        P.nsets = tex_in_bins ? 0 : 3;
        P.alpha_logit = d.alpha_logit; P.noise = noise_on ? in->noise_override : nullptr;
        P.noise_scale = noise_on ? d.opacity_noise : 0.f; P.thresh = thresh; P.nb = nb;
        P.alpha = FP(L.alpha); P.alpha_full = FP(L.alpha_full); P.keep = IP(L.keep);
        P.seed = d.seed; P.rng_step = in->rng_step;
        P.sq_eps = d.sq_eps; P.S = d.S; P.R6 = d.R6; P.T = d.T; P.trig = d.trig; P.nv = nv;
        P.ratio = d.ratio_block_scene; P.scale_min = d.scale_min; P.S_world = d.S_world; P.Rw = d.R_world; P.Tw = d.T_world;
        P.blk_verts = FP(L.blk_verts);
        P.sq_local = FP(L.sq_local);
        P.ground_base = d.ground_base; P.ngv = d.n_ground_verts; P.R6g = d.R6_ground; P.Tg = d.T_ground;
        P.ground_verts = d.env_verts + (size_t)d.n_sky_verts * 3;
        P.zero0 = d.small_grads; P.nzero0 = d.n_small_grads;
        if (phase == 1) { HIP_OK(hipMemsetAsync(d.small_grads, 0, (size_t)d.n_small_grads * 4, M)); P.nzero0 = 0; }
        RC(launch_step_prologue(P, M));
    } else {
        RC(dbw_posed_mesh_fwd(d.ground_base, d.n_ground_verts, d.R6_ground, d.T_ground, d.S_world, d.R_world, d.T_world,
                              d.env_verts + (size_t)d.n_sky_verts * 3, M));
        RC(dbw_texture_prep_fwd_sets(sets, 3, M));
        HIP_OK(hipMemsetAsync(d.small_grads, 0, (size_t)d.n_small_grads * 4, M));
        RC(dbw_block_alpha_fwd(d.alpha_logit, noise_on ? in->noise_override : nullptr, noise_on ? d.opacity_noise : 0.f, thresh, nb, FP(L.alpha),
                               FP(L.alpha_full), IP(L.keep), M));
        RC(dbw_sq_blocks_fwd(d.sq_eps, d.S, d.R6, d.T, d.trig, IP(L.keep), 0, nb, nv, d.ratio_block_scene, d.scale_min, d.S_world, d.R_world,
                             d.T_world, FP(L.blk_verts), M));
    }
    const bool prologue_signal_folded = flags && two && head && fused_setup && !setup_aside;
    if (two && head && !prologue_signal_folded) RC(signal(M, F_PROLOGUE, p->ev_prologue));
    int *cursor = nullptr;
    const uint32_t *blayout = nullptr;
    float *vals = FP(L.vals);
    auto side_head = [&]() -> int {
        if (two && head) RC(await(Rg, F_PROLOGUE, p->ev_prologue));

        if (bins) {
            const int64_t nsub = (int64_t)d.n_bins * DBW_BIN_SUBCURSORS;
            const double total_records = (double)d.n_bins * (double)L.bin_cap;
            cursor = IP(L.cursor[p->bin_turn]);
            if (head) HIP_OK(hipMemsetAsync(cursor, 0, (size_t)nsub * 4, Rg));
            if (p->bin_ready) {
                if (head) RC(dbw_bin_layout(IP(L.cursor[1 - p->bin_turn]), nsub, total_records, 64, (uint32_t *)(ws + L.layout[p->bin_turn]), Rg));
                blayout = (const uint32_t *)(ws + L.layout[p->bin_turn]);
            } else {
                if (head) RC(dbw_bin_layout(cursor, nsub, total_records, 1, (uint32_t *)(ws + L.layout_uniform), Rg));
                blayout = (const uint32_t *)(ws + L.layout_uniform);
            }
            if (two && head) RC(signal(Rg, F_LAYOUT, p->ev_layout));
        }
        if (!head) {
        } else if (d.fuse & 4) {
            RegulariserArgs A;
            memset(&A, 0, sizeof(A));
            A.u = overlap_on ? in->overlap_u_override : nullptr; A.npts = d.overlap_points; A.seed = d.seed; A.rng_step = in->rng_step;
            A.sq_eps = d.sq_eps; A.S = d.S; A.R6 = d.R6; A.T = d.T; A.alpha_full = FP(L.alpha_full); A.nb = nb;
            A.ratio = d.ratio_block_scene; A.scale_min = d.scale_min; A.inv_temp = overlap_on ? 1.f / d.overlap_temperature : 1.f; A.thresh = d.overlap_n_blocks;
            A.overlap_scale = d.w_overlap;
            A.pars_eps = 1e-6f; A.pars_scale = d.w_parsimony;
            A.loss_parsimony = vals + 1; A.loss_overlap = vals + 3;
            A.g_sq_eps = d.g_sq_eps; A.g_S = d.g_S; A.g_R6 = d.g_R6; A.g_T = d.g_T; A.g_alpha_full = FP(L.g_alpha_full);
            A.ws = FP(L.ovl_ws); A.ticket = (unsigned *)(ws + L.tickets);
            RC(launch_regularisers(A, Rg));
        } else {
            if (pars_on) RC(dbw_sqrt_mean(FP(L.alpha_full), nb, 1e-6f, d.w_parsimony, vals + 1, FP(L.g_alpha_full), Rg));
            if (overlap_on)
                RC(dbw_overlap_loss(in->overlap_u_override, d.overlap_points, d.sq_eps, d.S, d.R6, d.T, FP(L.alpha_full), nb, d.ratio_block_scene, d.scale_min,
                                    d.overlap_temperature, d.overlap_n_blocks, d.w_overlap, vals + 3, d.g_sq_eps, d.g_S, d.g_R6, d.g_T, FP(L.g_alpha_full),
                                    FP(L.ovl_ws), Rg));
        }
        if (tv) {
            add_tv_fields(L, ws, sets);
            if (head && tex_in_bins) RC(await(Rg, F_TEX, p->ev_prologue));
            if (head) RC(dbw_tv_l2sq_sets(sets, 3, vals + 2, Rg));
        }
        return DBW_OK;
    };
    if (!prologue_signal_folded) RC(side_head());

    if (!head) {
    } else if (fused_setup) {
        SceneSetupArgs A;
        memset(&A, 0, sizeof(A));
        A.R = in->R; A.T = in->T; A.Kmat = d.Kmat; A.B = B;
        SceneGeom &e = A.sc[0], &f = A.sc[1];
        e.verts = d.env_verts; e.faces = d.env_faces; e.V = Ve; e.F = Fe;
        f.verts = FP(L.blk_verts); f.faces = d.block_faces; f.V = Vf; f.F = Ff;
        const SceneBuf *sb[2] = {&L.e, &L.f};
        RasterWorkspace *rw[2] = {&we, &wf};
        for (int i = 0; i < 2; ++i) {
            SceneGeom &g = A.sc[i];
            g.cam_eps = d.cam_eps; g.zc_on = zc_on; g.zc = d.z_clip; g.persp = d.perspective_correct;
            g.fvc = FP(sb[i]->fvc); g.first_idx = IP(sb[i]->first); g.num_faces = IP(sb[i]->num); g.c2o = IP(sb[i]->c2o); g.neighbor = IP(sb[i]->nbr);
            g.code = IP(sb[i]->code); g.cw = FP(sb[i]->cw);
            g.bbox = rw[i]->bbox; g.recs = rw[i]->recs;
        }
        e.margin = 0.f; f.margin = margin_f;
        f.hdr = wf.hdr; f.nhdr = CELL_HDR_INTS;
        f.srec = wf.shade_recs; f.face_uvs = d.block_face_uvs; f.face_map = d.block_face_map; f.map_desc = d.block_map_desc; f.map_alpha = fa;
        SceneBinsArgs Bn;
        memset(&Bn, 0, sizeof(Bn));
        Bn.B = B; Bn.H = H; Bn.W = W; Bn.nx = wf.nx; Bn.ny = wf.ny;
        for (int i = 0; i < 2; ++i) {
            SceneBinsArgs::One &g = Bn.sc[i];
            g.bbox = rw[i]->bbox; g.recs = rw[i]->recs; g.first_idx = IP(sb[i]->first); g.num_faces = IP(sb[i]->num);
            g.list = rw[i]->list; g.count = rw[i]->count; g.mask = rw[i]->mask;
        }
        Bn.sc[1].cells = 1; Bn.sc[1].cell = wf.cell; Bn.sc[1].pool = wf.pool; Bn.sc[1].pool_cap = wf.pool_cap; Bn.sc[1].hdr = wf.hdr; Bn.sc[1].rank = wf.rank;
        if (fold) {
            e.hdr = we.hdr; e.nhdr = CELL_HDR_INTS;
            e.srec = we.shade_recs; e.face_uvs = d.env_face_uvs; e.face_map = d.env_face_map; e.map_desc = d.env_map_desc; e.map_alpha = nullptr;
            Bn.sc[0].cells = 1; Bn.sc[0].cell = we.cell; Bn.sc[0].pool = we.pool; Bn.sc[0].pool_cap = we.pool_cap; Bn.sc[0].hdr = we.hdr; Bn.sc[0].rank = we.rank;
            Bn.sc[0].dom = we.dom;
        }
        if (setup_aside) {
            RC(await(E, F_PROLOGUE, p->ev_prologue));
            A.scene0 = 0; A.nscenes = 1; Bn.scene0 = 0; Bn.nscenes = 1;
            RC(launch_scene_setup(A, M));
            RC(launch_scene_bins(Bn, M));
            A.scene0 = 1; Bn.scene0 = 1;
            RC(launch_scene_setup(A, E));
            RC(launch_scene_bins(Bn, E));
            RC(dbw_launch_work_scatter(wf, B, H, W, E));
            RC(signal(E, F_SCATTER, p->ev_scatter));
        } else {
            A.scene0 = 0; A.nscenes = 2; Bn.scene0 = 0; Bn.nscenes = 2;
            if (prologue_signal_folded) { A.sync_flag = p->sync_words + F_PROLOGUE; A.sync_val = ++p->sync_val[F_PROLOGUE]; }
            RC(launch_scene_setup(A, M));
            unsigned *tex_flag = nullptr, tex_val = 0;
            if (tex_in_bins) {
                for (int i = 0; i < 3; ++i) Bn.tex.s[i] = sets[i];
                Bn.tex.s[3] = sets[0];
                Bn.tex_sets = 3;
                const long long per = (long long)Bn.nx * Bn.ny * B;
                Bn.tex_z = (int)((2048 + per - 1) / per);
                tex_flag = p->sync_words + F_TEX; tex_val = ++p->sync_val[F_TEX];
            }
            RC(launch_scene_bins(Bn, M));
            RC(dbw_launch_work_scatter(wf, B, H, W, M, tex_flag, tex_val));
        }
    } else {
        RC(dbw_project_clip_fwd(d.env_verts, d.env_faces, in->R, in->T, d.Kmat, B, Ve, Fe, d.cam_eps, zc_on, d.z_clip, d.perspective_correct, FP(L.e.fvc),
                                IP(L.e.first), IP(L.e.num), IP(L.e.c2o), IP(L.e.nbr), IP(L.e.code), FP(L.e.cw), M));
        RC(dbw_project_clip_fwd(FP(L.blk_verts), d.block_faces, in->R, in->T, d.Kmat, B, Vf, Ff, d.cam_eps, zc_on, d.z_clip, d.perspective_correct,
                                FP(L.f.fvc), IP(L.f.first), IP(L.f.num), IP(L.f.c2o), IP(L.f.nbr), IP(L.f.code), FP(L.f.cw), M));
        RC(dbw_render_fwd_fused(FP(L.e.fvc), IP(L.e.first), IP(L.e.num), IP(L.e.nbr), IP(L.e.c2o), IP(L.e.code), FP(L.e.cw), 2 * Fe, d.env_face_uvs,
                                d.env_face_map, d.env_map_desc, FP(L.env_maps), nullptr, 0, B, Fte, H, W, 1, Fe, 0.f, 0.f, d.perspective_correct, d.bg_env,
                                IP(L.p2f_e), FP(L.bary_e), FP(L.dists_e), FP(L.img_e), ws + L.e.rws, L.e.rws_bytes, 3, 1, 1, M));
        RC(dbw_render_fwd_fused_mse(FP(L.f.fvc), IP(L.f.first), IP(L.f.num), IP(L.f.nbr), IP(L.f.c2o), IP(L.f.code), FP(L.f.cw), 2 * Ff, d.block_face_uvs,
                                    d.block_face_map, d.block_map_desc, FP(L.blk_maps), fa, alpha_len, B, Ftf, H, W, K, Ff, d.sigma, d.blur_radius,
                                    d.perspective_correct, d.bg_fg, IP(L.p2f), FP(L.bary), FP(L.dists), ws + L.f.rws, L.f.rws_bytes, nullptr, nullptr, 0.f,
                                    nullptr, nullptr, nullptr, 1, 1, M));
    }

    if (prologue_signal_folded) RC(side_head());

#define PROF(i, st) do { if (p->profile) HIP_OK(hipEventRecord(p->ev_t[i], st)); } while (0)
    PROF(0, M);
    if (!fold)
        RC(dbw_render_fwd_fused(FP(L.e.fvc), IP(L.e.first), IP(L.e.num), IP(L.e.nbr), IP(L.e.c2o), IP(L.e.code), FP(L.e.cw), 2 * Fe, d.env_face_uvs,
                                d.env_face_map, d.env_map_desc, FP(L.env_maps), nullptr, 0, B, Fte, H, W, 1, Fe, 0.f, 0.f, d.perspective_correct, d.bg_env,
                                IP(L.p2f_e), FP(L.bary_e), FP(L.dists_e), FP(L.img_e), ws + L.e.rws, L.e.rws_bytes, 3, 2, 1, M));
    PROF(1, M);
    if (setup_aside) RC(await(M, F_SCATTER, p->ev_scatter));
    PROF(2, M);
    if (fold) {
        EnvFoldHost fh;
        fh.ws = &we; fh.first_idx = IP(L.e.first); fh.num_faces = IP(L.e.num); fh.maps = FP(L.env_maps);
        for (int i = 0; i < 3; ++i) fh.bg[i] = d.bg_env[i];
        fh.p2f = IP(L.p2f_e); fh.uvj = FP(L.bary_e);
        RC(render_fwd_fused_mse_fold(FP(L.f.fvc), IP(L.f.first), IP(L.f.num), IP(L.f.nbr), IP(L.f.c2o), IP(L.f.code), FP(L.f.cw), 2 * Ff, d.block_face_uvs,
                                     d.block_face_map, d.block_map_desc, FP(L.blk_maps), fa, alpha_len, B, Ftf, H, W, K, Ff, d.sigma, d.blur_radius,
                                     d.perspective_correct, d.bg_fg, IP(L.p2f), FP(L.bary), FP(L.dists), ws + L.f.rws, L.f.rws_bytes, target, mse_scale,
                                     FP(L.part), FP(L.g_fg), FP(L.g_env), fh, phase == 1 ? in->rec_out : nullptr, phase == 2 ? in->grad_rec : nullptr, M));
        if (phase == 1) { p->phase1_done = true; return DBW_OK; }
        p->phase1_done = false;
    } else
    RC(dbw_render_fwd_fused_mse(FP(L.f.fvc), IP(L.f.first), IP(L.f.num), IP(L.f.nbr), IP(L.f.c2o), IP(L.f.code), FP(L.f.cw), 2 * Ff, d.block_face_uvs,
                                d.block_face_map, d.block_map_desc, FP(L.blk_maps), fa, alpha_len, B, Ftf, H, W, K, Ff, d.sigma, d.blur_radius,
                                d.perspective_correct, d.bg_fg, IP(L.p2f), FP(L.bary), FP(L.dists), ws + L.f.rws, L.f.rws_bytes, FP(L.img_e), target, mse_scale,
                                FP(L.part), FP(L.g_fg), FP(L.g_env), 2, 1, M));
    PROF(3, M);
    const bool seq = d.backward_order != 0 || (bins && !d.binned_concurrent);
    const bool fwd_signal_folded = flags && two;
    if (two && !fwd_signal_folded) RC(signal(M, F_FG_FWD, p->ev_fg_fwd));

    auto loss_values = [&](hipStream_t st) -> int {
        hipLaunchKernelGGL(loss_finish_kernel, dim3(LOSS_BLOCKS), dim3(256), 0, st, FP(L.part), (long long)B * L.tiles, mse_scale,
                           d.tv_value_scale != 0.f ? d.tv_value_scale : 1.f, vals, FP(L.losses));
        RC(dbw_check_launch("loss_finish_kernel"));
        if (two) RC(signal(st, F_REG, p->ev_reg));
        if (in->read_losses) {
            HIP_OK(hipMemcpyAsync(p->host_losses, FP(L.losses), 5 * sizeof(float), hipMemcpyDeviceToHost, st));
            HIP_OK(hipEventRecord(p->ev_losses, st));
            p->losses_pending = true;
        }
        return DBW_OK;
    };

    auto env_backward = [&](hipStream_t st) -> int {
        PROF(6, st);
        RC(dbw_render_bwd_fused(IP(L.p2f_e), FP(L.bary_e), FP(L.dists_e), IP(L.e.c2o), IP(L.e.code), FP(L.e.cw), 2 * Fe, d.env_face_uvs, d.env_face_map,
                                d.env_map_desc, FP(L.env_maps), nullptr, 0, B, H, W, 1, Fe, 0.f, d.bg_env, FP(L.g_env), FP(L.e.fvc), d.perspective_correct, 0,
                                FP(L.g_env_maps), nullptr, FP(L.g_fvc_e), 1, 3, nullptr, nullptr, nullptr, 0, nullptr, d.n_sky_faces, nullptr, 1, st));
        PROF(7, st);
        RC(dbw_project_clip_bwd(d.env_verts, d.env_faces, in->R, in->T, d.Kmat, B, Ve, Fe, d.cam_eps, d.z_clip, d.perspective_correct, IP(L.e.num),
                                IP(L.e.c2o), IP(L.e.code), FP(L.e.cw), FP(L.g_fvc_e), FP(L.g_env_verts), st));
        RC(dbw_posed_mesh_bwd(d.ground_base, d.n_ground_verts, d.R6_ground, d.T_ground, d.S_world, d.R_world, FP(L.g_env_verts) + (size_t)d.n_sky_verts * 3,
                              d.g_R6_ground, d.g_T_ground, st));
        if (defer || adam_tail) return DBW_OK;
        if (two) RC(await(st, F_REG, p->ev_reg));
        dbw_texture_set env_sets[2] = {sets[0], sets[2]};
        if (!tv) { env_sets[0].grad_sig = nullptr; env_sets[1].grad_sig = nullptr; }
        RC(dbw_texture_prep_bwd_sets(env_sets, 2, st));
        return DBW_OK;
    };
    auto side_after_fwd = [&]() -> int {
        if (two) {
            RC(await(Rg, F_FG_FWD, p->ev_fg_fwd));
            RC(loss_values(Rg));
        }
        if (two && !seq) {
            RC(await(E, F_FG_FWD, p->ev_fg_fwd));
            RC(env_backward(E));
            RC(signal(E, F_ENV_DONE, p->ev_env_done));
        }
        return DBW_OK;
    };
    if (!fwd_signal_folded) RC(side_after_fwd());

    if (bins && two) RC(await(M, F_LAYOUT, p->ev_layout));
    PROF(4, M);
    unsigned *bwd_flag = nullptr, bwd_val = 0;
    if (fwd_signal_folded) { bwd_flag = p->sync_words + F_FG_FWD; bwd_val = ++p->sync_val[F_FG_FWD]; }
    RC(render_bwd_fused_signal(IP(L.p2f), FP(L.bary), FP(L.dists), IP(L.f.c2o), IP(L.f.code), FP(L.f.cw), 2 * Ff, d.block_face_uvs, d.block_face_map,
                               d.block_map_desc, FP(L.blk_maps), fa, alpha_len, B, H, W, K, Ff, d.sigma, d.bg_fg, FP(L.g_fg), FP(L.f.fvc), d.perspective_correct, 1,
                               FP(L.g_blk_maps), coarse ? FP(L.g_fa) : nullptr, FP(L.g_fvc_f), d.decim_blocks > 1 ? 1 : 0, 2, bins ? d.block_bin_base : nullptr, cursor,
                               bins ? (void *)(ws + L.records) : nullptr, bins ? L.bin_cap : 0, blayout, 0, nullptr, 1, M, bwd_flag, bwd_val));
    PROF(5, M);
    if (fwd_signal_folded) RC(side_after_fwd());
    if (two && seq) {
        RC(signal(M, F_KERNEL_DONE, p->ev_kernel_done));
        RC(await(E, F_KERNEL_DONE, p->ev_kernel_done));
        RC(env_backward(E));
        RC(signal(E, F_ENV_DONE, p->ev_env_done));
    }
    if (bins) RC(dbw_texbin_reduce(d.block_bin_info, cursor, ws + L.records, L.bin_cap, blayout, d.n_bins, FP(L.g_blk_maps), M));
    if (adam_tail) RC(await(M, F_REG, p->ev_reg));
    const bool early_textures = two && !in->with_adam && !defer;
    auto blocks_textures = [&]() -> int {
        if (defer) return DBW_OK;
        dbw_texture_set blk = sets[1];
        if (!tv) blk.grad_sig = nullptr;
        RC(dbw_texture_prep_bwd_sets(&blk, 1, M));
        if (early_textures) RC(signal(M, F_BLOCKS_READY, p->ev_blocks_ready));
        return DBW_OK;
    };
    if (early_textures) {
        RC(await(M, F_REG, p->ev_reg));
        RC(blocks_textures());
    }
    const bool tail_merged = (d.fuse & 32) && !early_textures && !defer;
    if (!tail_merged)
        RC(dbw_project_clip_bwd(FP(L.blk_verts), d.block_faces, in->R, in->T, d.Kmat, B, Vf, Ff, d.cam_eps, d.z_clip, d.perspective_correct, IP(L.f.num),
                                IP(L.f.c2o), IP(L.f.code), FP(L.f.cw), FP(L.g_fvc_f), FP(L.g_blk_verts), M));
    if (!two) { RC(env_backward(M)); RC(loss_values(M)); }
    auto blocks_chain = [&]() -> int {
        if (tail_merged) {
            ClipBwdArgs C;
            C.verts = FP(L.blk_verts); C.faces = d.block_faces; C.R = in->R; C.T = in->T; C.Kmat = d.Kmat; C.B = B; C.V = Vf; C.F = Ff;
            C.eps = d.cam_eps; C.zc = d.z_clip; C.persp = d.perspective_correct;
            C.num_faces = IP(L.f.num); C.c2o = IP(L.f.c2o); C.code = IP(L.f.code); C.cw = FP(L.f.cw); C.gfvc = FP(L.g_fvc_f); C.gverts = FP(L.g_blk_verts);
            dbw_texture_set blk = sets[1];
            if (!tv) blk.grad_sig = nullptr;
            RC(launch_clip_bwd_tex(C, blk, M));
        } else if (!early_textures) RC(blocks_textures());
        if ((d.fuse & 8) && (d.fuse & 1)) {
            BlocksTailArgs A;
            memset(&A, 0, sizeof(A));
            A.sq_eps = d.sq_eps; A.S = d.S; A.R6 = d.R6; A.T = d.T; A.sq_local = FP(L.sq_local); A.keep = IP(L.keep); A.nb = nb; A.nv = nv;
            A.scale_min = d.scale_min; A.S_world = d.S_world; A.Rw = d.R_world; A.g_verts = FP(L.g_blk_verts);
            A.g_sq_eps = d.g_sq_eps; A.g_S = d.g_S; A.g_R6 = d.g_R6; A.g_T = d.g_T;
            A.alpha = FP(L.alpha); A.g_alpha_parts = coarse ? FP(L.g_fa) : nullptr; A.alpha_parts = 64; A.g_alpha_full = FP(L.g_alpha_full); A.g_logit = d.g_alpha_logit;
            if (!adam_tail) { A.void_raised = void_raised; A.void_flag = void_flag; }
            RC(launch_blocks_tail(A, M));
        } else {
            RC(dbw_sq_blocks_bwd(d.sq_eps, d.S, d.R6, d.T, d.trig, IP(L.keep), 0, nb, nv, d.ratio_block_scene, d.scale_min, d.S_world, d.R_world, FP(L.g_blk_verts),
                                 d.g_sq_eps, d.g_S, d.g_R6, d.g_T, M));
            RC(dbw_block_alpha_bwd(FP(L.alpha), IP(L.keep), coarse ? FP(L.g_fa) : nullptr, 64, FP(L.g_alpha_full), nb, d.g_alpha_logit, M));
            hipLaunchKernelGGL(void_latch_kernel, dim3(1), dim3(1), 0, M, (const float *)void_raised, void_flag);
            RC(dbw_check_launch("void_latch_kernel"));
        }
        return DBW_OK;
    };
    if (adam_tail) RC(blocks_chain());
    if (two) RC(await(M, F_ENV_DONE, p->ev_env_done));
    if (two && defer) RC(await(M, F_REG, p->ev_reg));
    if (!adam_tail) RC(blocks_chain());

    if (adam_tail) {
        T.tex[0] = sets[0]; T.tex[1] = sets[2];
        if (!tv) { T.tex[0].grad_sig = nullptr; T.tex[1].grad_sig = nullptr; }
        RC(launch_adam_tail(T, M));
        p->arena_clean = true;
        p->last_tail = true;
    } else if (in->with_adam) {
        p->last_tail = false;
        RC(dbw_adam_step_groups(d.flat_param, d.flat_grad, d.exp_avg, d.exp_avg_sq, d.group_end, in->lr, 2, in->beta1, in->beta2, in->adam_eps, in->adam_step,
                                ws + L.arena_begin, (int64_t)(L.arena_end - L.arena_begin), void_flag, M));
        p->arena_clean = true;
    }
    if (bins) { p->bin_turn = 1 - p->bin_turn; p->bin_ready = 1; }
    p->runs += 1;
    p->profiled = p->profile;
    return DBW_OK;
#undef PROF
#undef FP
#undef IP
}

extern "C" int dbw_train_step_finish(dbw_step_plan *p, const dbw_step_inputs *in, dbw_stream_t stream) {
    DBW_REQUIRE(p && in, "null pointer");
    DBW_REQUIRE(!in->with_adam || in->adam_step >= 1, "adam_step >= 1");
    const dbw_step_desc &d = p->d;
    const Layout &L = p->L;
    hipStream_t M = (hipStream_t)stream;
    dbw_texture_set sets[3];
    fill_texture_sets(d, L, p->ws, sets);
    if (tv_on(d)) add_tv_fields(L, p->ws, sets);
    RC(dbw_texture_prep_bwd_sets(sets, 3, M));
    if (in->with_adam) {
        RC(dbw_adam_step_groups(d.flat_param, d.flat_grad, d.exp_avg, d.exp_avg_sq, d.group_end, in->lr, 2, in->beta1, in->beta2, in->adam_eps, in->adam_step,
                                p->ws + L.arena_begin, (int64_t)(L.arena_end - L.arena_begin), (const float *)(p->ws + L.losses) + 7, M));
        p->arena_clean = true;
    }
    return DBW_OK;
}

extern "C" int dbw_train_step_wait_blocks_ready(dbw_step_plan *p, dbw_stream_t stream) {
    DBW_REQUIRE(p, "null pointer");
    if (!p->cur_flags) { HIP_OK(hipStreamWaitEvent((hipStream_t)stream, p->ev_blocks_ready, 0)); return DBW_OK; }
    hipLaunchKernelGGL(sync_wait_kernel, dim3(1), dim3(1), 0, (hipStream_t)stream, (const unsigned *)(p->sync_words + F_BLOCKS_READY), p->sync_val[F_BLOCKS_READY],
                       p->sync_words + SYNC_TIMEOUT_SLOT, p->host_timeouts_dev, (float *)(p->sync_words + SYNC_VOID_SLOT), SYNC_LIMIT_TICKS);
    return dbw_check_launch("sync_wait_kernel");
}

extern "C" int dbw_debug_train_step_force_timeout(dbw_step_plan *p) {
    if (!p) return DBW_ERR_INVALID;
    p->force_timeout = 1;
    return DBW_OK;
}
extern "C" int dbw_debug_train_step_hasty_prologue_wait(dbw_step_plan *p) {
    if (!p) return DBW_ERR_INVALID;
    p->force_timeout = 2;
    return DBW_OK;
}

extern "C" int dbw_debug_train_step_last_timeout(dbw_step_plan *p, int *out3) {
    DBW_REQUIRE(p && out3, "null pointer");
    unsigned w[3] = {0u, 0u, 0u};
    if (hipDeviceSynchronize() != hipSuccess || hipMemcpy(w, p->sync_words + SYNC_TIMEOUT_SLOT - 3, sizeof(w), hipMemcpyDeviceToHost) != hipSuccess) {
        dbw_set_error("dbw_debug_train_step_last_timeout: copy failed");
        return DBW_ERR_LAUNCH;
    }
    out3[0] = (int)w[0] - 1; out3[1] = (int)w[1]; out3[2] = (int)w[2];
    return DBW_OK;
}
extern "C" int dbw_debug_train_step_counters(dbw_step_plan *p, unsigned *seen12, unsigned *asked12) {
    DBW_REQUIRE(p && seen12 && asked12, "null pointer");
    unsigned first = 0u;
    if (hipDeviceSynchronize() != hipSuccess || hipMemcpy(&first, p->sync_words + SYNC_TIMEOUT_SLOT - 3, sizeof(first), hipMemcpyDeviceToHost) != hipSuccess ||
        hipMemcpy(seen12, p->sync_words + (first ? SYNC_TIMEOUT_SLOT + 1 : 0), SYNC_FLAGS * sizeof(unsigned), hipMemcpyDeviceToHost) != hipSuccess) {
        dbw_set_error("dbw_debug_train_step_counters: copy failed");
        return DBW_ERR_LAUNCH;
    }
    for (int i = 0; i < SYNC_FLAGS; ++i) asked12[i] = p->sync_val[i];
    return DBW_OK;
}
extern "C" int dbw_train_step_voided_runs(const dbw_step_plan *p) { return p ? p->voided_runs + (*(volatile unsigned *)p->host_timeouts != 0u ? 1 : 0) : -1; }

extern "C" int dbw_debug_train_step_last_tail(const dbw_step_plan *p) { return p ? (p->last_tail ? 1 : 0) : -1; }

extern "C" int64_t dbw_train_step_void_flag_offset(const dbw_step_plan *p) { return p ? (int64_t)p->L.losses + 7 * (int64_t)sizeof(float) : -1; }

extern "C" int dbw_train_step_sync_timeouts(dbw_step_plan *p) {
    if (!p) return -1;
    unsigned n = 0;
    if (hipDeviceSynchronize() != hipSuccess || hipMemcpy(&n, p->sync_words + SYNC_TIMEOUT_SLOT, sizeof(n), hipMemcpyDeviceToHost) != hipSuccess) return -1;
    return (int)n;
}

extern "C" int dbw_train_step_profile(dbw_step_plan *p, int on) {
    DBW_REQUIRE(p, "null pointer");
    p->profile = on != 0;
    p->profiled = false;
    return DBW_OK;
}

extern "C" int dbw_train_step_kernel_times(dbw_step_plan *p, float *out4_ms) {
    DBW_REQUIRE(p && out4_ms, "null pointer");
    DBW_REQUIRE(p->profiled, "no profiled run: dbw_train_step_profile(plan, 1), then a run");
    for (int k = 0; k < 4; ++k) {
        HIP_OK(hipEventSynchronize(p->ev_t[2 * k + 1]));
        HIP_OK(hipEventElapsedTime(out4_ms + k, p->ev_t[2 * k], p->ev_t[2 * k + 1]));
    }
    return DBW_OK;
}
```

Before: 78320 views/s.

## Fuse ground clip/pose backward into env tail kernel and fold block textures into Adam tail

Adds an env_tail_kernel that does the environment clip backward only for ground faces, accumulates ground vertex gradients in LDS, and has the last block (found via a ticket) compute the ground pose gradients. This replaces the separate clip-bwd and posed-mesh-bwd launches on the env stream. The Adam tail kernel is widened to handle a third texture set, so the block texture prep backward moves into the fused Adam tail. The block clip backward then runs as a plain kernel instead of the merged clip+texture kernel. The aim is fewer launches and less cross-stream serialization, at the cost of atomic contention and a last-block reduction running on a single wave.

```diff
diff --git a/differentiable-blocksworld_amd/csrc/project_clip.hip b/differentiable-blocksworld_amd/csrc/project_clip.hip
--- a/differentiable-blocksworld_amd/csrc/project_clip.hip
+++ b/differentiable-blocksworld_amd/csrc/project_clip.hip
@@ -1,10 +1,13 @@
 #include "dbw_common.h"
 #include "camera_math.h"
+#include "model_math.h"
 #include "shade_common.h"
 #include "raster_bin.h"
 #include "step_kernels.h"
 #include "texture_body.h"
 #include "../../include/dbw_hip.h"
+
+#include <string.h>
 
 using namespace dbw;
 
@@ -64,6 +67,49 @@
     if (tid == 0) { first_idx[b] = (int)base_out; num_faces[b] = running; }
 }
 
+__device__ __forceinline__ void clip_slot_bwd(const float *__restrict__ verts, const int *__restrict__ faces, const Cam &cam, float eps, float zc,
+                                              int persp, const int *__restrict__ c2o, const int *__restrict__ code, const float *__restrict__ cw,
+                                              long long o, const float (&g)[9], int &f, int (&vi)[3], float (&gw)[9]) {
+    f = c2o[o];
+    const int cd = code[o];
+    vi[0] = faces[f * 3]; vi[1] = faces[f * 3 + 1]; vi[2] = faces[f * 3 + 2];
+    f3 gv[3] = {{0.f, 0.f, 0.f}, {0.f, 0.f, 0.f}, {0.f, 0.f, 0.f}};
+    const f3 ga{g[0], g[1], g[2]}, gb{g[3], g[4], g[5]}, gc{g[6], g[7], g[8]};
+    if (cd < 0) {
+        gv[0] = ga; gv[1] = gb; gv[2] = gc;
+    } else {
+        const int i1 = cd & 3, kind = cd >> 2;
+        const f3 q0 = project(verts + (long long)vi[0] * 3, cam, eps).ndc, q1 = project(verts + (long long)vi[1] * 3, cam, eps).ndc,
+                 q2 = project(verts + (long long)vi[2] * 3, cam, eps).ndc;
+        const f3 P1 = i1 == 0 ? q0 : (i1 == 1 ? q1 : q2), P2 = i1 == 0 ? q1 : (i1 == 1 ? q2 : q0),
+                 P3 = i1 == 0 ? q2 : (i1 == 1 ? q0 : q1);
+        const float w2 = cw[o * 2], w3 = cw[o * 2 + 1];
+        f3 g1{0.f, 0.f, 0.f}, g2{0.f, 0.f, 0.f}, g3{0.f, 0.f, 0.f};
+        if (kind == 0) {
+            clip_point_bwd(P1, P2, zc, persp, w2, ga, g1, g2);
+            clip_point_bwd(P1, P3, zc, persp, w3, gb, g1, g3);
+            g1.x += gc.x; g1.y += gc.y; g1.z += gc.z;
+        } else if (kind == 1) {
+            clip_point_bwd(P1, P2, zc, persp, w2, ga, g1, g2);
+            g2.x += gb.x; g2.y += gb.y; g2.z += gb.z;
+            clip_point_bwd(P1, P3, zc, persp, w3, gc, g1, g3);
+        } else {
+            clip_point_bwd(P1, P3, zc, persp, w3, ga, g1, g3);
+            g2.x += gb.x; g2.y += gb.y; g2.z += gb.z;
+            g3.x += gc.x; g3.y += gc.y; g3.z += gc.z;
+        }
+        gv[0] = i1 == 0 ? g1 : (i1 == 1 ? g3 : g2);
+        gv[1] = i1 == 0 ? g2 : (i1 == 1 ? g1 : g3);
+        gv[2] = i1 == 0 ? g3 : (i1 == 1 ? g2 : g1);
+    }
+#pragma unroll
+    for (int i = 0; i < 3; ++i)
+        if (gv[i].x != 0.f || gv[i].y != 0.f || gv[i].z != 0.f) {
+            const f3 w = vertex_bwd(verts, vi[i], cam, eps, gv[i]);
+            gw[i * 3] = w.x; gw[i * 3 + 1] = w.y; gw[i * 3 + 2] = w.z;
+        }
+}
+
 constexpr int BWD_SLOTS = 8;
 template <bool LDS_TABLE>
 __device__ __forceinline__ void project_clip_bwd_body(
@@ -96,44 +142,7 @@
         if (act) {
             Cam cam;
             load_cam(R, T, Kmat, b, cam);
-            f = c2o[o];
-            const int cd = code[o];
-            vi[0] = faces[f * 3]; vi[1] = faces[f * 3 + 1]; vi[2] = faces[f * 3 + 2];
-            f3 gv[3] = {{0.f, 0.f, 0.f}, {0.f, 0.f, 0.f}, {0.f, 0.f, 0.f}};
-            const f3 ga{g[0], g[1], g[2]}, gb{g[3], g[4], g[5]}, gc{g[6], g[7], g[8]};
-            if (cd < 0) {
-                gv[0] = ga; gv[1] = gb; gv[2] = gc;
-            } else {
-                const int i1 = cd & 3, kind = cd >> 2;
-                const f3 q0 = project(verts + (long long)vi[0] * 3, cam, eps).ndc, q1 = project(verts + (long long)vi[1] * 3, cam, eps).ndc,
-                         q2 = project(verts + (long long)vi[2] * 3, cam, eps).ndc;
-                const f3 P1 = i1 == 0 ? q0 : (i1 == 1 ? q1 : q2), P2 = i1 == 0 ? q1 : (i1 == 1 ? q2 : q0),
-                         P3 = i1 == 0 ? q2 : (i1 == 1 ? q0 : q1);
-                const float w2 = cw[o * 2], w3 = cw[o * 2 + 1];
-                f3 g1{0.f, 0.f, 0.f}, g2{0.f, 0.f, 0.f}, g3{0.f, 0.f, 0.f};
-                if (kind == 0) {
-                    clip_point_bwd(P1, P2, zc, persp, w2, ga, g1, g2);
-                    clip_point_bwd(P1, P3, zc, persp, w3, gb, g1, g3);
-                    g1.x += gc.x; g1.y += gc.y; g1.z += gc.z;
-                } else if (kind == 1) {
-                    clip_point_bwd(P1, P2, zc, persp, w2, ga, g1, g2);
-                    g2.x += gb.x; g2.y += gb.y; g2.z += gb.z;
-                    clip_point_bwd(P1, P3, zc, persp, w3, gc, g1, g3);
-                } else {
-                    clip_point_bwd(P1, P3, zc, persp, w3, ga, g1, g3);
-                    g2.x += gb.x; g2.y += gb.y; g2.z += gb.z;
-                    g3.x += gc.x; g3.y += gc.y; g3.z += gc.z;
-                }
-                gv[0] = i1 == 0 ? g1 : (i1 == 1 ? g3 : g2);
-                gv[1] = i1 == 0 ? g2 : (i1 == 1 ? g1 : g3);
-                gv[2] = i1 == 0 ? g3 : (i1 == 1 ? g2 : g1);
-            }
-#pragma unroll
-            for (int i = 0; i < 3; ++i)
-                if (gv[i].x != 0.f || gv[i].y != 0.f || gv[i].z != 0.f) {
-                    const f3 w = vertex_bwd(verts, vi[i], cam, eps, gv[i]);
-                    gw[i * 3] = w.x; gw[i * 3 + 1] = w.y; gw[i * 3 + 2] = w.z;
-                }
+            clip_slot_bwd(verts, faces, cam, eps, zc, persp, c2o, code, cw, o, g, f, vi, gw);
         }
         const unsigned long long am = __ballot(act);
         if (am == 0ull) continue;
@@ -189,6 +198,71 @@
     else
         texture_prep_bwd_body(t.texture, t.n, t.h, t.w, t.decim, t.grad_maps, t.grad_sig, t.grad_texture, (long long)blockIdx.x - nclip,
                               (long long)gridDim.x - nclip);
+}
+
+constexpr int ENV_TAIL_MAX_BLOCKS = 256;
+__global__ __launch_bounds__(NT) void env_tail_kernel(const EnvTailArgs A) {
+    extern __shared__ float s_acc[];
+    __shared__ int s_last;
+    const ClipBwdArgs &C = A.clip;
+    const int tid = threadIdx.x, per = 2 * (C.F - A.face0), total = C.B * per;
+    for (int i = tid; i < A.ngv * 3; i += NT) s_acc[i] = 0.f;
+    __syncthreads();
+    for (int item = blockIdx.x * NT + tid; item < total; item += gridDim.x * NT) {
+        const int b = item / per, j = C.num_faces[b] - 1 - item % per;
+        if (j < 0) continue;
+        const long long o = (long long)b * 2 * C.F + j;
+        if (C.c2o[o] < A.face0) continue;
+        float g[9];
+        bool any = false;
+#pragma unroll
+        for (int i = 0; i < 9; ++i) { g[i] = C.gfvc[o * 9 + i]; any |= (g[i] != 0.f); }
+        if (!any) continue;
+        int f = -1, vi[3] = {0, 0, 0};
+        float gw[9] = {0.f, 0.f, 0.f, 0.f, 0.f, 0.f, 0.f, 0.f, 0.f};
+        Cam cam;
+        load_cam(C.R, C.T, C.Kmat, b, cam);
+        clip_slot_bwd(C.verts, C.faces, cam, C.eps, C.zc, C.persp, C.c2o, C.code, C.cw, o, g, f, vi, gw);
+#pragma unroll
+        for (int c = 0; c < 9; ++c)
+            if (gw[c] != 0.f) {
+                const int v = vi[c / 3] - A.vert0;
+                if (v >= 0 && v < A.ngv) atomicAdd(&s_acc[v * 3 + (c % 3)], gw[c]);
+                else unsafeAtomicAdd(C.gverts + (long long)vi[c / 3] * 3 + (c % 3), gw[c]);
+            }
+    }
+    __syncthreads();
+    float *gground = C.gverts + (long long)A.vert0 * 3;
+    for (int i = tid; i < A.ngv * 3; i += NT) {
+        const float v = s_acc[i];
+        if (v != 0.f) unsafeAtomicAdd(gground + i, v);
+    }
+    __threadfence();
+    __syncthreads();
+    if (tid == 0) s_last = atomicAdd(A.ticket, 1u) == gridDim.x - 1 ? 1 : 0;
+    __syncthreads();
+    if (!s_last) return;
+    __threadfence();
+    if (tid < DBW_WAVE) {
+        Pose p;
+        load_pose(nullptr, nullptr, A.R6, A.Tp, 0, 0.f, p);
+        float acc[17];
+#pragma unroll
+        for (int i = 0; i < 17; ++i) acc[i] = 0.f;
+        for (int v = tid; v < A.ngv; v += DBW_WAVE) {
+            float gin[3], gv[3];
+#pragma unroll
+            for (int i = 0; i < 3; ++i) gin[i] = __hip_atomic_load(gground + v * 3 + i, __ATOMIC_RELAXED, __HIP_MEMORY_SCOPE_AGENT);
+            pose_bwd(p, A.base + (long long)v * 3, A.S_world, A.Rw, gin, acc, gv);
+        }
+#pragma unroll
+        for (int i = 0; i < 17; ++i) acc[i] = wave_sum(acc[i]);
+        if (tid == 0) {
+            finish_pose_grads(p, nullptr, 0, acc, nullptr, nullptr, A.g_R6, A.g_T);
+            *A.ticket = 0u;
+            if (A.sync_flag) __hip_atomic_store(A.sync_flag, A.sync_val, __ATOMIC_RELEASE, __HIP_MEMORY_SCOPE_AGENT);
+        }
+    }
 }
 
 template <bool CACHED>
@@ -314,6 +388,23 @@
     return dbw_check_launch("clip_bwd_tex_kernel");
 }
 
+bool dbw::env_tail_fits(const EnvTailArgs &A) {
+    const ClipBwdArgs &C = A.clip;
+    return C.B > 0 && C.V > 0 && C.F > 0 && A.face0 >= 0 && A.face0 < C.F && A.vert0 >= 0 && A.ngv > 0 && A.vert0 + A.ngv <= C.V &&
+           (size_t)A.ngv * 3 * sizeof(float) <= 48 * 1024 && (long long)C.B * 2 * (C.F - A.face0) < 0x7fffffffLL - ENV_TAIL_MAX_BLOCKS * NT;
+}
+
+int dbw::launch_env_tail(const EnvTailArgs &A, hipStream_t s) {
+    const ClipBwdArgs &C = A.clip;
+    DBW_REQUIRE(C.verts && C.faces && C.R && C.T && C.Kmat && C.num_faces && C.c2o && C.code && C.cw && C.gfvc && C.gverts, "null pointer");
+    DBW_REQUIRE(A.base && A.R6 && A.Tp && A.Rw && A.g_R6 && A.g_T && A.ticket, "null pointer");
+    DBW_REQUIRE(env_tail_fits(A), "the ground's faces and vertices must be the mesh's last, its vertex gradients fit 48 KB of LDS");
+    const int total = C.B * 2 * (C.F - A.face0);
+    const int grid = min(ENV_TAIL_MAX_BLOCKS, (total + NT - 1) / NT);
+    hipLaunchKernelGGL(env_tail_kernel, dim3((unsigned)grid), dim3(NT), (size_t)A.ngv * 3 * sizeof(float), s, A);
+    return dbw_check_launch("env_tail_kernel");
+}
+
 int dbw::launch_scene_setup(const SceneSetupArgs &A, hipStream_t s) {
     DBW_REQUIRE(A.R && A.T && A.Kmat && A.B > 0, "bad argument");
     int chunks = 0;
@@ -332,6 +423,24 @@
     else
         hipLaunchKernelGGL(scene_setup_kernel<false>, dim3((unsigned)chunks, (unsigned)A.B, (unsigned)A.nscenes), dim3(NT), 0, s, A);
     return dbw_check_launch("scene_setup_kernel");
+}
+
+extern "C" int dbw_debug_env_tail(const float *verts_world, const int32_t *faces, const float *R, const float *T, const float *Kmat, int B, int V,
+                                  int F, float eps, float z_clip, int perspective_correct, const int32_t *num_faces, const int32_t *c2o,
+                                  const int32_t *clip_code, const float *clip_w, const float *grad_face_verts_c, float *grad_verts_world,
+                                  int first_ground_face, int first_ground_vert, int n_ground_verts, const float *ground_base, const float *R6,
+                                  const float *Tp, float S_world, const float *Rw, float *g_R6, float *g_T, unsigned *ticket,
+                                  unsigned *sync_flag, unsigned sync_val, dbw_stream_t stream) {
+    EnvTailArgs A;
+    memset(&A, 0, sizeof(A));
+    ClipBwdArgs &C = A.clip;
+    C.verts = verts_world; C.faces = faces; C.R = R; C.T = T; C.Kmat = Kmat; C.B = B; C.V = V; C.F = F; C.eps = eps; C.zc = z_clip;
+    C.persp = perspective_correct; C.num_faces = num_faces; C.c2o = c2o; C.code = clip_code; C.cw = clip_w; C.gfvc = grad_face_verts_c;
+    C.gverts = grad_verts_world;
+    A.face0 = first_ground_face; A.vert0 = first_ground_vert; A.ngv = n_ground_verts;
+    A.base = ground_base; A.R6 = R6; A.Tp = Tp; A.S_world = S_world; A.Rw = Rw; A.g_R6 = g_R6; A.g_T = g_T;
+    A.ticket = ticket; A.sync_flag = sync_flag; A.sync_val = sync_val;
+    return launch_env_tail(A, (hipStream_t)stream);
 }
 
 extern "C" int dbw_project_clip_fwd(const float *verts_world, const int32_t *faces, const float *R, const float *T,
diff --git a/differentiable-blocksworld_amd/csrc/step_kernels.h b/differentiable-blocksworld_amd/csrc/step_kernels.h
--- a/differentiable-blocksworld_amd/csrc/step_kernels.h
+++ b/differentiable-blocksworld_amd/csrc/step_kernels.h
@@ -87,11 +87,21 @@
 };
 int launch_clip_bwd_tex(const ClipBwdArgs &C, const dbw_texture_set &tex, hipStream_t s);
 
+struct EnvTailArgs {
+    ClipBwdArgs clip; int face0, vert0, ngv;
+    const float *base, *R6, *Tp; float S_world; const float *Rw;
+    float *g_R6, *g_T;
+    unsigned *ticket, *sync_flag; unsigned sync_val;
+};
+bool env_tail_fits(const EnvTailArgs &A);
+int launch_env_tail(const EnvTailArgs &A, hipStream_t s);
+
+constexpr int ADAM_TAIL_SETS = 3;
 struct AdamTailArgs {
     float *param, *grad, *exp_avg, *exp_avg_sq; const int64_t *group_end; const float *lr; int ngroups;
     float beta1, beta2, eps; int step;
     void *zero_buf; int64_t zero_bytes, hole_begin, hole_end;
-    dbw_texture_set tex[2]; int ntex;
+    dbw_texture_set tex[ADAM_TAIL_SETS]; int ntex;
     const float *void_raised; float *void_flag;
 };
 bool adam_tail_fits(const AdamTailArgs &A);
diff --git a/differentiable-blocksworld_amd/csrc/texture.hip b/differentiable-blocksworld_amd/csrc/texture.hip
--- a/differentiable-blocksworld_amd/csrc/texture.hip
+++ b/differentiable-blocksworld_amd/csrc/texture.hip
@@ -159,12 +159,12 @@
 struct AdamTailK {
     float *p, *g, *m, *v; long long n; AdamGroups G; float beta1, beta2, eps, bc2_sqrt;
     uint4 *zero_buf; long long zero_vec, hole_lo, hole_hi;
-    AdamTex t[2]; int ntex, clear_maps, nenv;
-    long long skip_lo[2], skip_len[2];
+    AdamTex t[ADAM_TAIL_SETS]; int ntex, clear_maps, nenv;
+    long long skip_lo[ADAM_TAIL_SETS], skip_len[ADAM_TAIL_SETS];
     const float *void_raised; float *void_flag;
 };
 
-__device__ __forceinline__ void adam_tex_set(const AdamTailK &A, const AdamTex &t, bool skip, long long etid, long long neth) {
+__device__ __forceinline__ void adam_tex_set(const AdamTailK &A, const AdamTex &t, bool skip, long long etid, long long neth, long long &rot) {
     if (t.d <= 1) {
         const long long total = (long long)t.n * t.h * t.w * 3;
         for (long long i = etid; i < total; i += neth) {
@@ -182,7 +182,11 @@
     const float inv = 1.f / (float)(t.d * t.d);
     const int ch_ = t.h / t.d, cw_ = t.w / t.d, lane = threadIdx.x & 63;
     const long long cells = (long long)t.n * ch_ * cw_;
-    for (long long c = etid >> 6; c < cells; c += neth >> 6) {
+    const long long nwaves = neth >> 6;
+    long long first = (etid >> 6) - rot % nwaves;
+    if (first < 0) first += nwaves;
+    rot += cells;
+    for (long long c = first; c < cells; c += nwaves) {
         const int m = (int)(c / ((long long)ch_ * cw_));
         const int r = (int)(c % ((long long)ch_ * cw_));
         const int cy = r / cw_, cx = r % cw_;
@@ -211,13 +215,17 @@
     const long long tid = (long long)blockIdx.x * blockDim.x + threadIdx.x, nth = (long long)gridDim.x * blockDim.x;
     const long long neth = (long long)A.nenv * blockDim.x;
     if (tid < neth) {
-        for (int k = 0; k < A.ntex; ++k) adam_tex_set(A, A.t[k], skip, tid, neth);
+        long long rot = 0;
+        for (int k = 0; k < A.ntex; ++k) adam_tex_set(A, A.t[k], skip, tid, neth, rot);
     } else if (!skip) {
-        const long long rest = A.n - A.skip_len[0] - A.skip_len[1];
+        long long rest = A.n;
+#pragma unroll
+        for (int k = 0; k < ADAM_TAIL_SETS; ++k) rest -= A.skip_len[k];
         for (long long j = tid - neth; j < rest; j += nth - neth) {
             long long i = j;
-            if (i >= A.skip_lo[0]) i += A.skip_len[0];
-            if (i >= A.skip_lo[1]) i += A.skip_len[1];
+#pragma unroll
+            for (int k = 0; k < ADAM_TAIL_SETS; ++k)
+                if (i >= A.skip_lo[k]) i += A.skip_len[k];
             adam_update(A.p[i], A.g[i], A.m[i], A.v[i], group_step_size(A.G, i), A.beta1, A.beta2, A.eps, A.bc2_sqrt);
         }
     }
@@ -359,11 +367,11 @@
 
 bool dbw::adam_tail_fits(const AdamTailArgs &A) {
     if (!A.param || !A.grad || !A.exp_avg || !A.exp_avg_sq || !A.group_end || !A.lr || !A.void_raised || A.ngroups < 1 || A.ngroups > MAX_SETS) return false;
-    if (A.ntex < 0 || A.ntex > 2 || A.zero_bytes < 0 || A.zero_bytes % 16 || ((uintptr_t)A.zero_buf & 15)) return false;
+    if (A.ntex < 0 || A.ntex > ADAM_TAIL_SETS || A.zero_bytes < 0 || A.zero_bytes % 16 || ((uintptr_t)A.zero_buf & 15)) return false;
     if (A.hole_begin < 0 || A.hole_begin > A.hole_end || A.hole_end > A.zero_bytes || A.hole_begin % 16 || A.hole_end % 16) return false;
     const long long n = A.group_end[A.ngroups - 1];
     const char *hb = (const char *)A.zero_buf + A.hole_begin, *he = (const char *)A.zero_buf + A.hole_end;
-    long long lo[2] = {0, 0}, hi[2] = {0, 0};
+    long long lo[ADAM_TAIL_SETS] = {0, 0, 0}, hi[ADAM_TAIL_SETS] = {0, 0, 0};
     for (int k = 0; k < A.ntex; ++k) {
         const dbw_texture_set &t = A.tex[k];
         if (!t.texture || !t.grad_maps || !t.grad_texture || t.n < 1 || t.h < 1 || t.w < 1 || t.decim < 1 || t.h % t.decim || t.w % t.decim) return false;
@@ -374,7 +382,10 @@
         const char *zb = (const char *)A.zero_buf, *ze = zb + A.zero_bytes;
         if (A.hole_end > A.hole_begin ? (mb < hb || me > he) : (mb < ze && me > zb)) return false;
     }
-    return A.ntex < 2 || hi[0] <= lo[1] || hi[1] <= lo[0];
+    for (int k = 1; k < A.ntex; ++k)
+        for (int q = 0; q < k; ++q)
+            if (!(hi[q] <= lo[k] || hi[k] <= lo[q])) return false;
+    return true;
 }
 
 int dbw::launch_adam_tail(const AdamTailArgs &A, hipStream_t s) {
@@ -395,14 +406,15 @@
     }
     K.void_raised = A.void_raised; K.void_flag = A.void_flag;
     long long env = 0;
-    for (int k = 0; k < 2; ++k) {
+    for (int k = 0; k < ADAM_TAIL_SETS; ++k) {
         K.skip_lo[k] = K.n; K.skip_len[k] = 0;
         if (k < A.ntex) { K.skip_lo[k] = K.t[k].off; K.skip_len[k] = (long long)K.t[k].n * K.t[k].h * K.t[k].w * 3; env += K.skip_len[k]; }
     }
-    if (K.skip_lo[1] < K.skip_lo[0]) {
-        std::swap(K.skip_lo[0], K.skip_lo[1]);
-        std::swap(K.skip_len[0], K.skip_len[1]);
-    }
+    for (int k = 1; k < ADAM_TAIL_SETS; ++k)
+        for (int q = k; q > 0 && K.skip_lo[q] < K.skip_lo[q - 1]; --q) {
+            std::swap(K.skip_lo[q], K.skip_lo[q - 1]);
+            std::swap(K.skip_len[q], K.skip_len[q - 1]);
+        }
     unsigned grid = grid_for(K.n);
     K.nenv = 0;
     if (A.ntex) {
@@ -415,11 +427,10 @@
     return dbw_check_launch("adam_groups_tex_kernel");
 }
 
-extern "C" int dbw_debug_adam_tail(float *param, float *grad, float *exp_avg, float *exp_avg_sq, const int64_t *group_end, const float *lr,
-                                   int ngroups, float beta1, float beta2, float eps, int step, void *zero_buf, int64_t zero_bytes,
-                                   int64_t hole_begin, int64_t hole_end, const dbw_texture_set *sets, int nsets, const float *void_raised,
-                                   float *void_flag, dbw_stream_t stream) {
-    DBW_REQUIRE(nsets >= 0 && nsets <= 2 && (sets || nsets == 0), "0..2 texture sets");
+static int debug_adam_tail(int max_sets, float *param, float *grad, float *exp_avg, float *exp_avg_sq, const int64_t *group_end, const float *lr, int ngroups,
+                           float beta1, float beta2, float eps, int step, void *zero_buf, int64_t zero_bytes, int64_t hole_begin, int64_t hole_end,
+                           const dbw_texture_set *sets, int nsets, const float *void_raised, float *void_flag, dbw_stream_t stream) {
+    DBW_REQUIRE(nsets >= 0 && nsets <= max_sets && (sets || nsets == 0), "too many texture sets");
     AdamTailArgs A;
     memset(&A, 0, sizeof(A));
     A.param = param; A.grad = grad; A.exp_avg = exp_avg; A.exp_avg_sq = exp_avg_sq; A.group_end = group_end; A.lr = lr; A.ngroups = ngroups;
@@ -428,6 +439,20 @@
     for (int k = 0; k < nsets; ++k) A.tex[k] = sets[k];
     A.ntex = nsets; A.void_raised = void_raised; A.void_flag = void_flag;
     return launch_adam_tail(A, (hipStream_t)stream);
+}
+extern "C" int dbw_debug_adam_tail(float *param, float *grad, float *exp_avg, float *exp_avg_sq, const int64_t *group_end, const float *lr,
+                                   int ngroups, float beta1, float beta2, float eps, int step, void *zero_buf, int64_t zero_bytes,
+                                   int64_t hole_begin, int64_t hole_end, const dbw_texture_set *sets, int nsets, const float *void_raised,
+                                   float *void_flag, dbw_stream_t stream) {
+    return debug_adam_tail(2, param, grad, exp_avg, exp_avg_sq, group_end, lr, ngroups, beta1, beta2, eps, step, zero_buf, zero_bytes, hole_begin, hole_end,
+                           sets, nsets, void_raised, void_flag, stream);
+}
+extern "C" int dbw_debug_adam_tail_sets(float *param, float *grad, float *exp_avg, float *exp_avg_sq, const int64_t *group_end, const float *lr,
+                                        int ngroups, float beta1, float beta2, float eps, int step, void *zero_buf, int64_t zero_bytes,
+                                        int64_t hole_begin, int64_t hole_end, const dbw_texture_set *sets, int nsets, const float *void_raised,
+                                        float *void_flag, dbw_stream_t stream) {
+    return debug_adam_tail(ADAM_TAIL_SETS, param, grad, exp_avg, exp_avg_sq, group_end, lr, ngroups, beta1, beta2, eps, step, zero_buf, zero_bytes, hole_begin,
+                           hole_end, sets, nsets, void_raised, void_flag, stream);
 }
 
 extern "C" int dbw_composite_mse(const float *fg, const float *env, const float *imgs, int N, int H, int W,
diff --git a/differentiable-blocksworld_amd/csrc/train_step.hip b/differentiable-blocksworld_amd/csrc/train_step.hip
--- a/differentiable-blocksworld_amd/csrc/train_step.hip
+++ b/differentiable-blocksworld_amd/csrc/train_step.hip
@@ -259,6 +259,8 @@
 }
 constexpr unsigned long long SYNC_LIMIT_TICKS = 100000000ull;
 
+constexpr long long BLOCKS_IN_ADAM_MAX_FLOATS = 4ll << 20;
+
 }
 
 struct dbw_step_plan {
@@ -283,6 +285,7 @@
     int voided_runs;
     int force_timeout;
     bool last_tail;
+    int tail_form;
 };
 
 extern "C" size_t dbw_train_step_workspace_bytes(const dbw_step_desc *desc) {
@@ -335,7 +338,7 @@
     for (hipEvent_t &e : p->ev_t)
         if (hipEventCreate(&e) != hipSuccess) { dbw_set_error("dbw_train_step_create: hipEventCreate failed"); dbw_train_step_destroy(p); return nullptr; }
     p->runs = 0; p->cur_flags = false; p->voided_runs = 0; p->force_timeout = 0; p->bin_turn = 0; p->bin_ready = 0; p->uniform_ready = 0; p->arena_clean = false; p->losses_pending = false;
-    p->last_tail = false;
+    p->last_tail = false; p->tail_form = 0;
     return p;
 }
 
@@ -473,6 +476,24 @@
     T.void_raised = void_raised; T.void_flag = void_flag;
     const bool adam_tail = in->with_adam && !defer && (d.fuse & 41) == 41 && two && in->B > d.serial_setup_max_views && !bins_on(d) &&
                            adam_tail_fits(T);
+    AdamTailArgs T3 = T;
+    T3.tex[2] = sets[1]; T3.ntex = 3;
+    T3.hole_begin = (int64_t)(L.g_blk_maps - L.arena_begin);
+    EnvTailArgs Et;
+    memset(&Et, 0, sizeof(Et));
+    {
+        ClipBwdArgs &C = Et.clip;
+        C.verts = d.env_verts; C.faces = d.env_faces; C.R = in->R; C.T = in->T; C.Kmat = d.Kmat; C.B = in->B; C.V = L.Ve; C.F = L.Fe;
+        C.eps = d.cam_eps; C.zc = d.z_clip; C.persp = d.perspective_correct;
+        C.num_faces = (const int *)(ws + L.e.num); C.c2o = (const int *)(ws + L.e.c2o); C.code = (const int *)(ws + L.e.code);
+        C.cw = (const float *)(ws + L.e.cw); C.gfvc = (const float *)(ws + L.g_fvc_e); C.gverts = (float *)(ws + L.g_env_verts);
+        Et.face0 = d.n_sky_faces; Et.vert0 = d.n_sky_verts; Et.ngv = d.n_ground_verts;
+        Et.base = d.ground_base; Et.R6 = d.R6_ground; Et.Tp = d.T_ground; Et.S_world = d.S_world; Et.Rw = d.R_world;
+        Et.g_R6 = d.g_R6_ground; Et.g_T = d.g_T_ground;
+        Et.ticket = (unsigned *)(ws + L.tickets) + 1;
+    }
+    const bool short_tail = adam_tail && (d.fuse & 1) && (long long)d.n_blocks * d.txt_size * d.txt_size * 3 <= BLOCKS_IN_ADAM_MAX_FLOATS &&
+                            adam_tail_fits(T3) && env_tail_fits(Et);
 
     const float *target = in->imgs;
     if (!in->imgs_tiled) {
@@ -703,6 +724,12 @@
                                 d.env_map_desc, FP(L.env_maps), nullptr, 0, B, H, W, 1, Fe, 0.f, d.bg_env, FP(L.g_env), FP(L.e.fvc), d.perspective_correct, 0,
                                 FP(L.g_env_maps), nullptr, FP(L.g_fvc_e), 1, 3, nullptr, nullptr, nullptr, 0, nullptr, d.n_sky_faces, nullptr, 1, st));
         PROF(7, st);
+        if (short_tail) {
+            if (flags) { Et.sync_flag = p->sync_words + F_ENV_DONE; Et.sync_val = ++p->sync_val[F_ENV_DONE]; }
+            RC(launch_env_tail(Et, st));
+            if (!flags) HIP_OK(hipEventRecord(p->ev_env_done, st));
+            return DBW_OK;
+        }
         RC(dbw_project_clip_bwd(d.env_verts, d.env_faces, in->R, in->T, d.Kmat, B, Ve, Fe, d.cam_eps, d.z_clip, d.perspective_correct, IP(L.e.num),
                                 IP(L.e.c2o), IP(L.e.code), FP(L.e.cw), FP(L.g_fvc_e), FP(L.g_env_verts), st));
         RC(dbw_posed_mesh_bwd(d.ground_base, d.n_ground_verts, d.R6_ground, d.T_ground, d.S_world, d.R_world, FP(L.g_env_verts) + (size_t)d.n_sky_verts * 3,
@@ -722,7 +749,7 @@
         if (two && !seq) {
             RC(await(E, F_FG_FWD, p->ev_fg_fwd));
             RC(env_backward(E));
-            RC(signal(E, F_ENV_DONE, p->ev_env_done));
+            if (!short_tail) RC(signal(E, F_ENV_DONE, p->ev_env_done));
         }
         return DBW_OK;
     };
@@ -742,7 +769,7 @@
         RC(signal(M, F_KERNEL_DONE, p->ev_kernel_done));
         RC(await(E, F_KERNEL_DONE, p->ev_kernel_done));
         RC(env_backward(E));
-        RC(signal(E, F_ENV_DONE, p->ev_env_done));
+        if (!short_tail) RC(signal(E, F_ENV_DONE, p->ev_env_done));
     }
     if (bins) RC(dbw_texbin_reduce(d.block_bin_info, cursor, ws + L.records, L.bin_cap, blayout, d.n_bins, FP(L.g_blk_maps), M));
     if (adam_tail) RC(await(M, F_REG, p->ev_reg));
@@ -765,7 +792,10 @@
                                 IP(L.f.c2o), IP(L.f.code), FP(L.f.cw), FP(L.g_fvc_f), FP(L.g_blk_verts), M));
     if (!two) { RC(env_backward(M)); RC(loss_values(M)); }
     auto blocks_chain = [&]() -> int {
-        if (tail_merged) {
+        if (tail_merged && short_tail) {
+            RC(dbw_project_clip_bwd(FP(L.blk_verts), d.block_faces, in->R, in->T, d.Kmat, B, Vf, Ff, d.cam_eps, d.z_clip, d.perspective_correct, IP(L.f.num),
+                                    IP(L.f.c2o), IP(L.f.code), FP(L.f.cw), FP(L.g_fvc_f), FP(L.g_blk_verts), M));
+        } else if (tail_merged) {
             ClipBwdArgs C;
             C.verts = FP(L.blk_verts); C.faces = d.block_faces; C.R = in->R; C.T = in->T; C.Kmat = d.Kmat; C.B = B; C.V = Vf; C.F = Ff;
             C.eps = d.cam_eps; C.zc = d.z_clip; C.persp = d.perspective_correct;
@@ -798,13 +828,17 @@
     if (!adam_tail) RC(blocks_chain());
 
     if (adam_tail) {
+        if (short_tail) T = T3;
         T.tex[0] = sets[0]; T.tex[1] = sets[2];
-        if (!tv) { T.tex[0].grad_sig = nullptr; T.tex[1].grad_sig = nullptr; }
+        if (short_tail) T.tex[2] = sets[1];
+        if (!tv) { T.tex[0].grad_sig = nullptr; T.tex[1].grad_sig = nullptr; T.tex[2].grad_sig = nullptr; }
         RC(launch_adam_tail(T, M));
         p->arena_clean = true;
         p->last_tail = true;
+        p->tail_form = short_tail ? 2 : 1;
     } else if (in->with_adam) {
         p->last_tail = false;
+        p->tail_form = 0;
         RC(dbw_adam_step_groups(d.flat_param, d.flat_grad, d.exp_avg, d.exp_avg_sq, d.group_end, in->lr, 2, in->beta1, in->beta2, in->adam_eps, in->adam_step,
                                 ws + L.arena_begin, (int64_t)(L.arena_end - L.arena_begin), void_flag, M));
         p->arena_clean = true;
@@ -880,6 +914,8 @@
 
 extern "C" int dbw_debug_train_step_last_tail(const dbw_step_plan *p) { return p ? (p->last_tail ? 1 : 0) : -1; }
 
+extern "C" int dbw_debug_train_step_tail_form(const dbw_step_plan *p) { return p ? p->tail_form : -1; }
+
 extern "C" int64_t dbw_train_step_void_flag_offset(const dbw_step_plan *p) { return p ? (int64_t)p->L.losses + 7 * (int64_t)sizeof(float) : -1; }
 
 extern "C" int dbw_train_step_sync_timeouts(dbw_step_plan *p) {
```

After: 76890 views/s. 0.982x the previous value.
